# skygazer42/realtime-video-analytics-32streams

Measured on AMD Instinct MI355X. Metric: aggregate detected FPS across streams + p99 per-frame latency, 32x1080p30, higher is better.
Workload: dtype f16

## Files before the change

### include/rva.h

```cpp
#ifndef RVA_H
#define RVA_H

#include <stdint.h>

#ifdef __cplusplus
extern "C" {
#endif

#define RVA_ABI_VERSION 1

enum rva_status {
    RVA_OK = 0,
    RVA_ERR_ARG = 1,
    RVA_ERR_HIP = 2,
    RVA_ERR_CAPACITY = 3,
    RVA_ERR_UNAVAILABLE = 4
};

enum rva_dtype { RVA_F16 = 0, RVA_F32 = 1, RVA_F64 = 2  };

typedef struct rva_ctx rva_ctx;
typedef struct rva_tracker rva_tracker;
typedef void *rva_stream_t;

// ... 147 lines not shown

int rva_sppf_pool3_nhwc_f16(rva_ctx *ctx, const void *in, int ldi, void *out1, void *out2, void *out3, int ldo,
                            int batch, int H, int W, int C, rva_stream_t stream);
int rva_maxpool5_nhwc_f16(rva_ctx *ctx, const void *in, int ldi, void *out, int ldo, int batch, int H,
                          int W, int C, rva_stream_t stream);
int rva_upsample2x_nhwc_f16(rva_ctx *ctx, const void *in, int ldi, void *out, int ldo, int batch, int H,
                            int W, int C, rva_stream_t stream);
int rva_yolo_head_f16(rva_ctx *ctx, const void *box_logits, int ldb, const void *cls_logits, int ldc,
                      void *out, int batch, int h, int w, int nc, int anchors_total, int anchor_offset,
                      float stride, rva_stream_t stream);
int rva_yolo_head3_f16(rva_ctx *ctx, const void *const *box_logits, const int32_t *ldb, const void *const *cls_logits,
                       const int32_t *ldc, void *out, int batch, const int32_t *h, const int32_t *w, int nc,
                       int anchors_total, const float *strides, rva_stream_t stream);
int rva_yolo_head_box32_f16(rva_ctx *ctx, const void *box_logits, int ldb, const void *cls_logits, int ldc, void *out,
                            float *boxes32, int batch, int h, int w, int nc, int anchors_total, int anchor_offset, float stride,
                            rva_stream_t stream);
int rva_yolo_head3_box32_f16(rva_ctx *ctx, const void *const *box_logits, const int32_t *ldb, const void *const *cls_logits,
                             const int32_t *ldc, void *out, float *boxes32, int batch, const int32_t *h, const int32_t *w, int nc,
                             int anchors_total, const float *strides, rva_stream_t stream);
int rva_yolo_head_nc_f16(rva_ctx *ctx, const void *box_logits, int ldb, const void *cls_logits, int ldc, void *out,
                         float *boxes32, int batch, int h, int w, int nc, int anchors_total, int anchor_offset, float stride,
                         rva_stream_t stream);
int rva_yolo_head3_nc_f16(rva_ctx *ctx, const void *const *box_logits, const int32_t *ldb, const void *const *cls_logits,
                          const int32_t *ldc, void *out, float *boxes32, int batch, const int32_t *h, const int32_t *w, int nc,
                          int anchors_total, const float *strides, rva_stream_t stream);
int rva_conv1x1_head_nc_f16(rva_ctx *ctx, const void *in, int ldi, const void *weights, const float *bias, int batch,
                            int H, int W, int Cin, int Cout, int mode, void *out, float *boxes32, int nc, int anchors_total,
                            int anchor_offset, float stride_px, int variant, rva_stream_t stream);

int rva_conv_f32_num_variants(void);
int rva_conv2d_nhwc_f32_v(rva_ctx *ctx, const void *in, int ldi, const void *weights, const float *bias,
                          void *out, int ldo, const void *residual, int ldr, int batch, int H, int W, int Cin,
                          int Cout, int ksize, int stride, int act, int variant, rva_stream_t stream);
int rva_stem_conv_f32(rva_ctx *ctx, const void *in_planar, const void *weights, const float *bias,
                      void *out, int ldo, int batch, int H, int W, int Cout, rva_stream_t stream);
int rva_maxpool5_nhwc_f32(rva_ctx *ctx, const void *in, int ldi, void *out, int ldo, int batch, int H,
                          int W, int C, rva_stream_t stream);
int rva_upsample2x_nhwc_f32(rva_ctx *ctx, const void *in, int ldi, void *out, int ldo, int batch, int H,
                            int W, int C, rva_stream_t stream);
int rva_yolo_head_f32(rva_ctx *ctx, const void *box_logits, int ldb, const void *cls_logits, int ldc,
                      void *out, int batch, int h, int w, int nc, int anchors_total, int anchor_offset,
                      float stride, rva_stream_t stream);

#define RVA_PLAN_NO_STEM2 1
#define RVA_PLAN_NO_CIN_PAD 2
#define RVA_PLAN_NO_PAIR32 4
#define RVA_PLAN_F32 8
#define RVA_PLAN_BOX_F32 16
typedef struct rva_yolov8_plan rva_yolov8_plan;
typedef struct rva_yolov8_desc {
    int32_t batch, height, width;
    int32_t widths[5];
    int32_t depth_backbone[4];
    int32_t depth_head;
    int32_t nc, reg_max;
    int32_t n_convs;
    int32_t flags;
} rva_yolov8_desc;
typedef struct rva_conv_weights {
    const float *weight;
    const float *bias;
    int32_t cout, cin, k, stride;
} rva_conv_weights;
int rva_yolov8_plan_create(rva_ctx *ctx, const rva_yolov8_desc *desc, const rva_conv_weights *convs, rva_yolov8_plan **out);
void rva_yolov8_plan_destroy(rva_yolov8_plan *plan);
int rva_yolov8_plan_info(const rva_yolov8_plan *plan, int32_t *anchors, int32_t *out_rows, int32_t *n_steps, int32_t *n_tunable,
                         int32_t *quiet_step);
int rva_yolov8_plan_output_layout(const rva_yolov8_plan *plan, int64_t *total_bytes, int64_t *boxes_offset);
int rva_yolov8_plan_run(rva_yolov8_plan *plan, const void *input, void *output, rva_stream_t stream);
int rva_yolov8_plan_run_lanes(rva_yolov8_plan *plan, const void *input, void *output, rva_stream_t stream, rva_stream_t side1,
                              rva_stream_t side2);
int rva_yolov8_plan_run_range(rva_yolov8_plan *plan, const void *input, void *output, int first, int last, rva_stream_t stream);
int rva_yolov8_plan_tunable_desc(const rva_yolov8_plan *plan, int index, char *buf, int len);
int rva_yolov8_plan_launch_tunable(rva_yolov8_plan *plan, int index, int variant, void *output, rva_stream_t stream);
int rva_yolov8_plan_set_variant(rva_yolov8_plan *plan, int index, int variant);
int rva_yolov8_plan_get_variant(const rva_yolov8_plan *plan, int index);
int rva_yolov8_plan_set_static_rows(rva_yolov8_plan *plan, int top, int bottom);
int rva_yolov8_plan_run_n(rva_yolov8_plan *plan, const void *input, void *output, int n, rva_stream_t stream);
int rva_yolov8_plan_run_lanes_n(rva_yolov8_plan *plan, const void *input, void *output, int n, rva_stream_t stream, rva_stream_t side1,
                                rva_stream_t side2);
int rva_yolov8_plan_run_range_n(rva_yolov8_plan *plan, const void *input, void *output, int n, int first, int last, rva_stream_t stream);
int rva_yolov8_plan_primed_images(const rva_yolov8_plan *plan);
int rva_yolov8_plan_step_rows(const rva_yolov8_plan *plan, int step, int32_t *y0, int32_t *y1);
int rva_yolov8_plan_step_desc(const rva_yolov8_plan *plan, int step, char *buf, int len);

typedef struct rva_yolov5_desc {
    int32_t batch, height, width;
    int32_t widths[5];
    int32_t depth_backbone[4];
    int32_t depth_head;
    int32_t nc;
    float anchors[18];
    int32_t n_convs;
    int32_t flags;
} rva_yolov5_desc;
int rva_yolov5_plan_create(rva_ctx *ctx, const rva_yolov5_desc *desc, const rva_conv_weights *convs, rva_yolov8_plan **out);
int rva_stem6_conv_f16(rva_ctx *ctx, const void *in_planar, const void *weights, const float *bias, void *out, int ldo,
                       int batch, int H, int W, int Cout, rva_stream_t stream);
int rva_stem6_conv_f16_rows(rva_ctx *ctx, const void *in_planar, const void *weights, const float *bias, void *out, int ldo,
                            int batch, int H, int W, int Cout, int y0, int y1, rva_stream_t stream);
int rva_conv_rows_through_pad(int k, int stride, int pad, int H_in, int lo, int hi, int32_t *out_lo, int32_t *out_hi);
int rva_conv1x1_head5_f16(rva_ctx *ctx, const void *in, int ldi, const void *weights, const float *bias, int batch, int H, int W,
                          int Cin, int nc, const float *anchors_px, void *out, float *boxes32, int anchors_total, int anchor_offset,
                          float stride_px, int variant, rva_stream_t stream);

typedef struct rva_yolo11_desc {
    int32_t batch, height, width;
    int32_t widths[5];
    int32_t repeats[8];
    int32_t c3k[8];
    int32_t psa_blocks, psa_heads;
    int32_t nc;
    int32_t n_convs;
    int32_t flags;
} rva_yolo11_desc;
int rva_yolo11_plan_create(rva_ctx *ctx, const rva_yolo11_desc *desc, const rva_conv_weights *convs, rva_yolov8_plan **out);
int rva_dwconv3x3_nhwc_f16(rva_ctx *ctx, const void *in, int ldi, const void *weights, const float *bias, void *out, int ldo,
                           const void *residual, int ldr, int batch, int H, int W, int C, int act, rva_stream_t stream);
int rva_psa_attention_f16(rva_ctx *ctx, const void *qkv, int ld, void *out, int ldo, int batch, int tokens, int heads,
                          rva_stream_t stream);

typedef struct rva_cnnlstm_plan rva_cnnlstm_plan;
typedef struct rva_cnnlstm_desc {
    int32_t height, width;
    int32_t frames;
    int32_t hidden, classes;
    int32_t max_clips;
} rva_cnnlstm_desc;
typedef struct rva_cnnlstm_weights {
    const float *conv1_w, *conv1_b, *conv2_w, *conv2_b;
    const float *w_ih1, *b1, *w_hh1;
    const float *w_ih2, *w_hh2, *b2;
    const float *head_w, *head_b;
} rva_cnnlstm_weights;
int rva_cnnlstm_plan_create(rva_ctx *ctx, const rva_cnnlstm_desc *desc, const rva_cnnlstm_weights *weights, rva_cnnlstm_plan **out);
void rva_cnnlstm_plan_destroy(rva_cnnlstm_plan *plan);
int rva_cnnlstm_plan_info(const rva_cnnlstm_plan *plan, int32_t *pooled_h, int32_t *pooled_w, int32_t *conv2_tiles,
                          int32_t *n_launches);
int rva_cnnlstm_plan_run(rva_cnnlstm_plan *plan, const void *frames, const int32_t *frame_index, int n_clips, void *logits,
                         rva_stream_t stream);
int rva_cnnlstm_plan_run_post(rva_cnnlstm_plan *plan, const void *logits, const int32_t *rows, int n_rows, int max_det,
                              void *scores, void *cls, void *boxes, void *counts, rva_stream_t stream);
enum rva_cnnlstm_stage {
    RVA_CNNLSTM_STAGE_POOLED = 0, RVA_CNNLSTM_STAGE_PARTIAL = 1, RVA_CNNLSTM_STAGE_FEAT = 2, RVA_CNNLSTM_STAGE_GX = 3,
    RVA_CNNLSTM_STAGE_H1 = 4, RVA_CNNLSTM_STAGE_H2 = 5
};
int rva_cnnlstm_plan_stage(rva_cnnlstm_plan *plan, int stage, int n_clips, void *dst, int64_t dst_floats, int64_t *n_floats,
                           rva_stream_t stream);

typedef struct rva_cnnlstm_f16_plan rva_cnnlstm_f16_plan;
int rva_cnnlstm_f16_plan_create(rva_ctx *ctx, const rva_cnnlstm_desc *desc, const rva_cnnlstm_weights *weights,
                                rva_cnnlstm_f16_plan **out);
void rva_cnnlstm_f16_plan_destroy(rva_cnnlstm_f16_plan *plan);
int rva_cnnlstm_f16_plan_info(const rva_cnnlstm_f16_plan *plan, int32_t *pooled_h, int32_t *pooled_w, int32_t *conv2_tiles,
                              int32_t *n_launches);
int rva_cnnlstm_f16_plan_run(rva_cnnlstm_f16_plan *plan, const void *frames, const int32_t *frame_index, int n_clips, void *logits,
                             rva_stream_t stream);
int rva_cnnlstm_f16_plan_run_post(rva_cnnlstm_f16_plan *plan, const void *logits, const int32_t *rows, int n_rows, int max_det,
                                  void *scores, void *cls, void *boxes, void *counts, rva_stream_t stream);
int rva_cnnlstm_f16_plan_stage(rva_cnnlstm_f16_plan *plan, int stage, int n_clips, void *dst, int64_t dst_elems, int64_t *n_elems,
                               rva_stream_t stream);

typedef struct rva_cnn3d_plan rva_cnn3d_plan;
typedef struct rva_cnn3d_desc {
    int32_t height, width;
    int32_t frames;
// ... 180 lines not shown
```

### realtime_video_analytics_32streams_amd/_native.py

```python
from __future__ import annotations

import ctypes as C
import os
import shutil
import subprocess
from pathlib import Path
from typing import Optional

PKG = Path(__file__).resolve().parent
ROOT = PKG.parent
CSRC = PKG / "csrc"
LIB_PATH = Path(os.environ["RVA_LIB_PATH"]) if os.environ.get("RVA_LIB_PATH") else PKG / "librva.so"
SOURCES = ["rva_ctx.hip", "rva_preprocess.hip", "rva_postprocess.hip", "rva_tracker.hip", "rva_conv.hip", "rva_stem.hip", "rva_yolo_ops.hip", "rva_conv_f32.hip", "rva_attn.hip", "rva_plan.hip", "rva_clip.hip",
           "rva_clip3d.hip", "rva_clip_f16.hip", "rva_resnet.hip", "rva_resnet_f16.hip", "rva_gates.hip", "rva_decode.hip", "rva_preview.hip", "rva_jpeg.hip", "rva_jpeg_dec.hip"]
HIPCC_FLAGS = ["--offload-arch=gfx950", "-O3", "-fPIC", "-shared", "-std=c++17", "-ffp-contract=off",
               "-Wall", "-Wno-unused-function"]

RVA_OK, RVA_ERR_ARG, RVA_ERR_HIP, RVA_ERR_CAPACITY, RVA_ERR_UNAVAILABLE = range(5)
RVA_F16, RVA_F32, RVA_F64 = 0, 1, 2
NORM_IMAGENET_F32, NORM_VIDEO_F32, NORM_IMAGENET_F64 = 0, 1, 2
LAYOUT_NCHW, LAYOUT_CNHW = 0, 1
RVA_MAX_BATCH = 64
RVA_CODEC_H264, RVA_CODEC_HEVC = 0, 1
RVA_JPEG_DEC_BGR, RVA_JPEG_DEC_NV12 = 0, 1
RVA_JPEG_DEC_OK, RVA_JPEG_DEC_REFUSED, RVA_JPEG_DEC_FAILED = 0, -1, -2


class Letterbox(C.Structure):
    _fields_ = [("src_w", C.c_int32), ("src_h", C.c_int32), ("dst_w", C.c_int32), ("dst_h", C.c_int32),
                ("new_w", C.c_int32), ("new_h", C.c_int32), ("pad_left", C.c_int32), ("pad_top", C.c_int32),
                ("scale", C.c_double)]

    def as_meta(self) -> dict:
        return {"orig_shape": (self.src_h, self.src_w), "scale": self.scale, "pad": (self.pad_left, self.pad_top)}


class YoloV8Desc(C.Structure):
    _fields_ = [("batch", C.c_int32), ("height", C.c_int32), ("width", C.c_int32), ("widths", C.c_int32 * 5),
                ("depth_backbone", C.c_int32 * 4), ("depth_head", C.c_int32), ("nc", C.c_int32), ("reg_max", C.c_int32),
                ("n_convs", C.c_int32), ("flags", C.c_int32)]


class YoloV5Desc(C.Structure):
    _fields_ = [("batch", C.c_int32), ("height", C.c_int32), ("width", C.c_int32), ("widths", C.c_int32 * 5),
                ("depth_backbone", C.c_int32 * 4), ("depth_head", C.c_int32), ("nc", C.c_int32), ("anchors", C.c_float * 18),
                ("n_convs", C.c_int32), ("flags", C.c_int32)]


class Yolo11Desc(C.Structure):
    _fields_ = [("batch", C.c_int32), ("height", C.c_int32), ("width", C.c_int32), ("widths", C.c_int32 * 5),
                ("repeats", C.c_int32 * 8), ("c3k", C.c_int32 * 8), ("psa_blocks", C.c_int32), ("psa_heads", C.c_int32),
                ("nc", C.c_int32), ("n_convs", C.c_int32), ("flags", C.c_int32)]


class ConvWeights(C.Structure):
    _fields_ = [("weight", C.POINTER(C.c_float)), ("bias", C.POINTER(C.c_float)), ("cout", C.c_int32), ("cin", C.c_int32),
                ("k", C.c_int32), ("stride", C.c_int32)]


class CnnLstmDesc(C.Structure):
    _fields_ = [("height", C.c_int32), ("width", C.c_int32), ("frames", C.c_int32), ("hidden", C.c_int32), ("classes", C.c_int32),
                ("max_clips", C.c_int32)]


class CnnLstmWeights(C.Structure):
    NAMES = ("conv1_w", "conv1_b", "conv2_w", "conv2_b", "w_ih1", "b1", "w_hh1", "w_ih2", "w_hh2", "b2", "head_w", "head_b")
    _fields_ = [(n, C.POINTER(C.c_float)) for n in NAMES]


class Cnn3dDesc(C.Structure):
    _fields_ = [("height", C.c_int32), ("width", C.c_int32), ("frames", C.c_int32), ("classes", C.c_int32), ("max_clips", C.c_int32)]


class Cnn3dWeights(C.Structure):
    NAMES = ("conv1_w", "conv1_b", "conv2_w", "conv2_b", "conv3_w", "conv3_b", "head_w", "head_b")
    _fields_ = [(n, C.POINTER(C.c_float)) for n in NAMES]


class ResNetDesc(C.Structure):
    _fields_ = [("height", C.c_int32), ("width", C.c_int32), ("classes", C.c_int32), ("top_k", C.c_int32), ("max_frames", C.c_int32)]


class ResNetWeights(C.Structure):
    NAMES = ("stem_w", "stem_b") + tuple(f"c{i}_{x}" for i in range(19) for x in "wb") + ("head_w", "head_b")
    _fields_ = [(n, C.POINTER(C.c_float)) for n in NAMES]


class ResNetConv(C.Structure):
    _fields_ = [("w", C.POINTER(C.c_float)), ("b", C.POINTER(C.c_float))]


class ResNetXDesc(C.Structure):
    _fields_ = [("height", C.c_int32), ("width", C.c_int32), ("classes", C.c_int32), ("top_k", C.c_int32), ("max_frames", C.c_int32),
                ("bottleneck", C.c_int32), ("blocks", C.c_int32 * 4), ("n_convs", C.c_int32), ("flags", C.c_int32)]


# ... 103 lines not shown
        "rva_tracker_update_gated_f32": (C.c_int, [_P, i32p, _P, _P, _P, _P, C.c_int, C.c_double, _P, i32p, _P]),
        "rva_tracker_set_gates": (C.c_int, [_P, i32p, i32p, i32p, i32p, C.c_int]),
        "rva_tracker_snapshot_status": (C.c_int, [_P, C.c_int, _P, _P, C.POINTER(C.c_int32)]),
        "rva_tracker_new_counts": (_P, [_P]),
        "rva_tracker_assign_ids": (C.c_int, [_P, _P, C.c_int, i32p, _P]),
        "rva_tracker_read": (C.c_int, [_P, C.c_int, C.c_int, _P, _P, _P, _P, _P, _P, _P, i32p, _P]),
        "rva_tracker_read_all": (C.c_int, [_P, _P, _P, _P, _P, _P, _P, _P, _P, _P]),
        "rva_tracker_snapshot_async": (C.c_int, [_P, C.c_int, _P]),
        "rva_tracker_snapshot_fetch": (C.c_int, [_P, C.c_int, C.c_int, _P, _P, _P, _P, _P, _P, _P, _P]),
        "rva_tracker_state": (C.c_int, [_P, i64p, C.POINTER(C.c_int), _P]),
        "rva_tracker_set_next_id": (C.c_int, [_P, C.c_int64, _P]),
        "rva_preview_nv12": (C.c_int, [_P, _P, _P, C.c_int, C.c_int, C.c_int, C.c_int, _P, C.c_int, C.c_int, _P, _P, C.c_int, _P, C.c_int,
                                       C.c_int, _P]),
        "rva_decode_available": (C.c_int, [C.c_char_p, C.c_int]),
        "rva_decoder_create": (C.c_int, [_P, C.c_int, C.c_int, C.POINTER(_P)]),
        "rva_decoder_destroy": (None, [_P]),
        "rva_decoder_feed": (C.c_int, [_P, C.c_char_p, C.c_int, C.c_int64, C.c_int]),
        "rva_decoder_next_frame": (C.c_int, [_P, C.POINTER(_P), C.POINTER(_P), i32p, i32p, i32p, i64p, i32p]),
        "rva_decoder_release": (C.c_int, [_P, C.c_int]),
        "rva_motion_nv12_batch": (C.c_int, [_P, pp, pp, i32p, pp, pp, C.c_int, C.c_int, C.c_int, _P, _P]),
        "rva_motion_nv12_masked_batch": (C.c_int, [_P, pp, pp, i32p, pp, pp, pp, C.c_int, C.c_int, C.c_int, _P, _P]),
        "rva_motion_bgr_batch": (C.c_int, [_P, pp, i32p, pp, pp, C.c_int, C.c_int, C.c_int, _P, _P]),
        "rva_preprocess_nv12_masked_batch": (C.c_int, [_P, pp, pp, i32p, pp, C.c_int, C.c_int, C.c_int, _P, C.c_int, C.c_int,
                                                       C.c_int, C.POINTER(Letterbox), _P]),
        "rva_resize_nv12_to_bgr_batch": (C.c_int, [_P, pp, pp, i32p, pp, C.c_int, C.c_int, C.c_int, _P, C.c_int, C.c_int, _P]),
        "rva_tracker_set_box_scale": (C.c_int, [_P, f64p]),
        "rva_conv_cout_pad": (C.c_int, [C.c_int]),
        "rva_conv_num_variants": (C.c_int, []),
        "rva_conv_variant_name": (C.c_char_p, [C.c_int]),
        "rva_conv2d_nhwc_f16": (C.c_int, [_P, _P, C.c_int, _P, _P, _P, C.c_int, _P, C.c_int] + [C.c_int] * 8 + [_P]),
        "rva_conv2d_nhwc_f16_v": (C.c_int, [_P, _P, C.c_int, _P, _P, _P, C.c_int, _P, C.c_int] + [C.c_int] * 9 + [_P]),
        "rva_conv2d_nhwc_f16_rows": (C.c_int, [_P, _P, C.c_int, _P, _P, _P, C.c_int, _P, C.c_int] + [C.c_int] * 11 + [_P]),
        "rva_conv_rows_through": (C.c_int, [C.c_int] * 5 + [i32p, i32p]),
        "rva_stem2_f16_rows": (C.c_int, [_P, _P, _P, _P, _P, _P, _P, C.c_int, C.c_int, C.c_int, C.c_int, C.c_int, C.c_int, _P]),
        "rva_stem_conv_f16": (C.c_int, [_P, _P, _P, _P, _P, C.c_int, C.c_int, C.c_int, C.c_int, C.c_int, _P]),
        "rva_stem2_f16": (C.c_int, [_P, _P, _P, _P, _P, _P, _P, C.c_int, C.c_int, C.c_int, C.c_int, _P]),
        "rva_c2f_pair32_f16": (C.c_int, [_P, _P, C.c_int, _P, _P, _P, _P, _P, C.c_int, C.c_int, C.c_int, C.c_int, _P]),
        "rva_conv1x1_head_f16": (C.c_int, [_P, _P, C.c_int, _P, _P, C.c_int, C.c_int, C.c_int, C.c_int, C.c_int, C.c_int, _P, C.c_int,
                                           C.c_int, C.c_int, C.c_float, C.c_int, _P]),
        "rva_conv1x1_head_box32_f16": (C.c_int, [_P, _P, C.c_int, _P, _P, C.c_int, C.c_int, C.c_int, C.c_int, _P, _P, C.c_int,
                                                 C.c_int, C.c_int, C.c_float, C.c_int, _P]),
        "rva_yolo_head_box32_f16": (C.c_int, [_P, _P, C.c_int, _P, C.c_int, _P, _P, C.c_int, C.c_int, C.c_int, C.c_int, C.c_int,
                                              C.c_int, C.c_float, _P]),
        "rva_yolo_head3_box32_f16": (C.c_int, [_P, pp, i32p, pp, i32p, _P, _P, C.c_int, i32p, i32p, C.c_int, C.c_int,
                                               C.POINTER(C.c_float), _P]),
        "rva_yolo_head_nc_f16": (C.c_int, [_P, _P, C.c_int, _P, C.c_int, _P, _P, C.c_int, C.c_int, C.c_int, C.c_int, C.c_int,
                                           C.c_int, C.c_float, _P]),
        "rva_yolo_head3_nc_f16": (C.c_int, [_P, pp, i32p, pp, i32p, _P, _P, C.c_int, i32p, i32p, C.c_int, C.c_int,
                                            C.POINTER(C.c_float), _P]),
        "rva_conv1x1_head_nc_f16": (C.c_int, [_P, _P, C.c_int, _P, _P, C.c_int, C.c_int, C.c_int, C.c_int, C.c_int, C.c_int, _P, _P,
                                              C.c_int, C.c_int, C.c_int, C.c_float, C.c_int, _P]),
        "rva_conv1x1_upcat_f16": (C.c_int, [_P, _P, C.c_int, C.c_int, _P, C.c_int, C.c_int, _P, _P, _P, C.c_int, C.c_int, C.c_int,
                                            C.c_int, C.c_int, C.c_int, C.c_int, _P]),
        "rva_yolo_head3_f16": (C.c_int, [_P, pp, i32p, pp, i32p, _P, C.c_int, i32p, i32p, C.c_int, C.c_int, C.POINTER(C.c_float), _P]),
        "rva_sppf_pool3_nhwc_f16": (C.c_int, [_P, _P, C.c_int, _P, _P, _P, C.c_int, C.c_int, C.c_int, C.c_int, C.c_int, _P]),
        "rva_maxpool5_nhwc_f16": (C.c_int, [_P, _P, C.c_int, _P, C.c_int, C.c_int, C.c_int, C.c_int, C.c_int, _P]),
        "rva_upsample2x_nhwc_f16": (C.c_int, [_P, _P, C.c_int, _P, C.c_int, C.c_int, C.c_int, C.c_int, C.c_int, _P]),
        "rva_yolo_head_f16": (C.c_int, [_P, _P, C.c_int, _P, C.c_int, _P, C.c_int, C.c_int, C.c_int, C.c_int, C.c_int,
                                        C.c_int, C.c_float, _P]),
        "rva_conv_f32_num_variants": (C.c_int, []),
        "rva_conv2d_nhwc_f32_v": (C.c_int, [_P, _P, C.c_int, _P, _P, _P, C.c_int, _P, C.c_int] + [C.c_int] * 9 + [_P]),
        "rva_stem_conv_f32": (C.c_int, [_P, _P, _P, _P, _P, C.c_int, C.c_int, C.c_int, C.c_int, C.c_int, _P]),
        "rva_maxpool5_nhwc_f32": (C.c_int, [_P, _P, C.c_int, _P, C.c_int, C.c_int, C.c_int, C.c_int, C.c_int, _P]),
        "rva_upsample2x_nhwc_f32": (C.c_int, [_P, _P, C.c_int, _P, C.c_int, C.c_int, C.c_int, C.c_int, C.c_int, _P]),
        "rva_yolo_head_f32": (C.c_int, [_P, _P, C.c_int, _P, C.c_int, _P, C.c_int, C.c_int, C.c_int, C.c_int, C.c_int,
                                        C.c_int, C.c_float, _P]),
        "rva_yolov8_plan_create": (C.c_int, [_P, C.POINTER(YoloV8Desc), C.POINTER(ConvWeights), C.POINTER(_P)]),
        "rva_yolov8_plan_destroy": (None, [_P]),
        "rva_yolov8_plan_info": (C.c_int, [_P, i32p, i32p, i32p, i32p, i32p]),
        "rva_yolov8_plan_output_layout": (C.c_int, [_P, i64p, i64p]),
        "rva_yolov8_plan_run": (C.c_int, [_P, _P, _P, _P]),
        "rva_yolov8_plan_run_lanes": (C.c_int, [_P, _P, _P, _P, _P, _P]),
        "rva_yolov8_plan_run_range": (C.c_int, [_P, _P, _P, C.c_int, C.c_int, _P]),
        "rva_yolov8_plan_tunable_desc": (C.c_int, [_P, C.c_int, C.c_char_p, C.c_int]),
        "rva_yolov8_plan_launch_tunable": (C.c_int, [_P, C.c_int, C.c_int, _P, _P]),
        "rva_yolov8_plan_set_variant": (C.c_int, [_P, C.c_int, C.c_int]),
        "rva_yolov8_plan_get_variant": (C.c_int, [_P, C.c_int]),
        "rva_yolov8_plan_set_static_rows": (C.c_int, [_P, C.c_int, C.c_int]),
        "rva_yolov8_plan_step_rows": (C.c_int, [_P, C.c_int, i32p, i32p]),
        "rva_yolov8_plan_run_n": (C.c_int, [_P, _P, _P, C.c_int, _P]),
        "rva_yolov8_plan_run_lanes_n": (C.c_int, [_P, _P, _P, C.c_int, _P, _P, _P]),
        "rva_yolov8_plan_run_range_n": (C.c_int, [_P, _P, _P, C.c_int, C.c_int, C.c_int, _P]),
        "rva_yolov8_plan_primed_images": (C.c_int, [_P]),
        "rva_yolov5_plan_create": (C.c_int, [_P, C.POINTER(YoloV5Desc), C.POINTER(ConvWeights), C.POINTER(_P)]),
        "rva_stem6_conv_f16": (C.c_int, [_P, _P, _P, _P, _P, C.c_int, C.c_int, C.c_int, C.c_int, C.c_int, _P]),
        "rva_stem6_conv_f16_rows": (C.c_int, [_P, _P, _P, _P, _P, C.c_int, C.c_int, C.c_int, C.c_int, C.c_int, C.c_int, C.c_int, _P]),
        "rva_conv_rows_through_pad": (C.c_int, [C.c_int] * 6 + [i32p, i32p]),
        "rva_conv1x1_head5_f16": (C.c_int, [_P, _P, C.c_int, _P, _P, C.c_int, C.c_int, C.c_int, C.c_int, C.c_int, _P, _P, _P,
                                            C.c_int, C.c_int, C.c_float, C.c_int, _P]),
        "rva_yolov8_plan_step_desc": (C.c_int, [_P, C.c_int, C.c_char_p, C.c_int]),
        "rva_yolo11_plan_create": (C.c_int, [_P, C.POINTER(Yolo11Desc), C.POINTER(ConvWeights), C.POINTER(_P)]),
        "rva_dwconv3x3_nhwc_f16": (C.c_int, [_P, _P, C.c_int, _P, _P, _P, C.c_int, _P, C.c_int] + [C.c_int] * 5 + [_P]),
        "rva_psa_attention_f16": (C.c_int, [_P, _P, C.c_int, _P, C.c_int, C.c_int, C.c_int, C.c_int, _P]),
        "rva_cnnlstm_plan_create": (C.c_int, [_P, C.POINTER(CnnLstmDesc), C.POINTER(CnnLstmWeights), C.POINTER(_P)]),
        "rva_cnnlstm_plan_destroy": (None, [_P]),
        "rva_cnnlstm_plan_info": (C.c_int, [_P, i32p, i32p, i32p, i32p]),
        "rva_cnnlstm_plan_run": (C.c_int, [_P, _P, _P, C.c_int, _P, _P]),
        "rva_cnnlstm_plan_run_post": (C.c_int, [_P, _P, _P, C.c_int, C.c_int, _P, _P, _P, _P, _P]),
        "rva_cnnlstm_plan_stage": (C.c_int, [_P, C.c_int, C.c_int, _P, C.c_int64, i64p, _P]),
        "rva_cnnlstm_f16_plan_create": (C.c_int, [_P, C.POINTER(CnnLstmDesc), C.POINTER(CnnLstmWeights), C.POINTER(_P)]),
        "rva_cnnlstm_f16_plan_destroy": (None, [_P]),
        "rva_cnnlstm_f16_plan_info": (C.c_int, [_P, i32p, i32p, i32p, i32p]),
        "rva_cnnlstm_f16_plan_run": (C.c_int, [_P, _P, _P, C.c_int, _P, _P]),
        "rva_cnnlstm_f16_plan_run_post": (C.c_int, [_P, _P, _P, C.c_int, C.c_int, _P, _P, _P, _P, _P]),
        "rva_cnnlstm_f16_plan_stage": (C.c_int, [_P, C.c_int, C.c_int, _P, C.c_int64, i64p, _P]),
        "rva_cnn3d_plan_create": (C.c_int, [_P, C.POINTER(Cnn3dDesc), C.POINTER(Cnn3dWeights), C.POINTER(_P)]),
        "rva_cnn3d_plan_destroy": (None, [_P]),
        "rva_cnn3d_plan_info": (C.c_int, [_P, i32p, i32p, i32p, i32p]),
        "rva_cnn3d_plan_run": (C.c_int, [_P, _P, _P, C.c_int, _P, _P]),
        "rva_cnn3d_plan_run_post": (C.c_int, [_P, _P, _P, C.c_int, C.c_int, _P, _P, _P, _P, _P]),
        "rva_cnn3d_plan_stage": (C.c_int, [_P, C.c_int, C.c_int, _P, C.c_int64, i64p, _P]),
        "rva_cnn3d_f16_plan_create": (C.c_int, [_P, C.POINTER(Cnn3dDesc), C.POINTER(Cnn3dWeights), C.POINTER(_P)]),
        "rva_cnn3d_f16_plan_destroy": (None, [_P]),
        "rva_cnn3d_f16_plan_info": (C.c_int, [_P, i32p, i32p, i32p, i32p]),
        "rva_cnn3d_f16_plan_run": (C.c_int, [_P, _P, _P, C.c_int, _P, _P]),
        "rva_cnn3d_f16_plan_run_post": (C.c_int, [_P, _P, _P, C.c_int, C.c_int, _P, _P, _P, _P, _P]),
        "rva_cnn3d_f16_plan_stage": (C.c_int, [_P, C.c_int, C.c_int, _P, C.c_int64, i64p, _P]),
        "rva_resnet_plan_create": (C.c_int, [_P, C.POINTER(ResNetDesc), C.POINTER(ResNetWeights), C.POINTER(_P)]),
        "rva_resnet_plan_destroy": (None, [_P]),
        "rva_resnet_plan_info": (C.c_int, [_P, i32p, i64p, i32p]),
        "rva_resnet_plan_run": (C.c_int, [_P, _P, _P, C.c_int, _P, _P]),
        "rva_resnet_plan_run_post": (C.c_int, [_P, _P, _P, C.c_int, C.c_int, _P, _P, _P, _P, _P]),
        "rva_resnet_plan_stage": (C.c_int, [_P, C.c_int, C.c_int, _P, C.c_int64, i64p, _P]),
        "rva_resnet_f16_plan_create": (C.c_int, [_P, C.POINTER(ResNetDesc), C.POINTER(ResNetWeights), C.POINTER(_P)]),
        "rva_resnet_f16_plan_destroy": (None, [_P]),
        "rva_resnet_f16_plan_info": (C.c_int, [_P, i32p, i64p, i32p]),
        "rva_resnet_f16_plan_run": (C.c_int, [_P, _P, _P, C.c_int, _P, _P]),
        "rva_resnet_f16_plan_run_post": (C.c_int, [_P, _P, _P, C.c_int, C.c_int, _P, _P, _P, _P, _P]),
        "rva_resnet_f16_plan_stage": (C.c_int, [_P, C.c_int, C.c_int, _P, C.c_int64, i64p, _P]),
        "rva_resnetx_f16_plan_create": (C.c_int, [_P, C.POINTER(ResNetXDesc), C.POINTER(ResNetXWeights), C.POINTER(_P)]),
        "rva_resnetx_f16_plan_destroy": (None, [_P]),
        "rva_resnetx_f16_plan_info": (C.c_int, [_P, i32p, i64p, i32p]),
        "rva_resnetx_f16_plan_run": (C.c_int, [_P, _P, _P, C.c_int, _P, _P]),
        "rva_resnetx_f16_plan_run_post": (C.c_int, [_P, _P, _P, C.c_int, C.c_int, _P, _P, _P, _P, _P]),
        "rva_resnetx_f16_plan_stage": (C.c_int, [_P, C.c_int, C.c_int, _P, C.c_int64, i64p, _P]),
        "rva_jpeg_max_bytes": (C.c_int, [C.c_int, C.c_int]),
        "rva_jpeg_encode_bgr": (C.c_int, [_P, _P, C.c_int, C.c_int, C.c_int, C.c_int, _P, C.c_int, _P, _P]),
        "rva_jpeg_status": (C.c_int, [_P, _P, C.POINTER(C.c_int)]),
        "rva_jpeg_batch_create": (C.c_int, [_P, C.c_int, C.c_int, C.c_int, C.POINTER(_P)]),
        "rva_jpeg_batch_destroy": (None, [_P]),
        "rva_jpeg_batch_encode": (C.c_int, [_P, C.c_int, pp, i32p, i32p, i32p, i32p, _P, C.c_int64, _P, _P]),
        "rva_preview_nv12_batch": (C.c_int, [_P, _P, _P, C.c_int64, C.c_int, C.c_int, C.c_int, C.c_int, _P]),
        "rva_jpeg_dec_probe": (C.c_int, [C.c_char_p, C.c_int64, C.POINTER(JpegDecInfo), C.c_char_p, C.c_int]),
        "rva_jpeg_dec_create": (C.c_int, [_P, C.c_int, C.c_int, C.c_int, C.c_int, C.POINTER(_P)]),
        "rva_jpeg_dec_destroy": (None, [_P]),
        "rva_jpeg_dec_decode": (C.c_int, [_P, C.c_int, C.POINTER(C.c_char_p), i64p, C.c_int, pp, pp, i32p, _P]),
        "rva_jpeg_dec_status": (C.c_int, [_P, i32p]),
        "rva_jpeg_dec_times": (C.c_int, [_P, f32p]),
    }
    for name, (res, args) in sig.items():
        fn = getattr(L, name)
        fn.restype = res
        fn.argtypes = args
    if L.rva_abi_version() != 1:
        raise RuntimeError("librva.so ABI version mismatch; rebuild it")
    _LIB = L
    return L


EXPORTS = [
    "rva_abi_version", "rva_create", "rva_destroy", "rva_last_error", "rva_reserve", "rva_letterbox_meta",
    "rva_preprocess_nv12_batch", "rva_preprocess_nv12_content_batch", "rva_preprocess_bgr_batch", "rva_preprocess_clip_nv12_batch",
    "rva_preprocess_clip_bgr_batch", "rva_profile_next_preprocess", "rva_preprocess_frames_nv12_batch", "rva_preprocess_frames_bgr_batch", "rva_postprocess_batch", "rva_post_status", "rva_post_filter_stats", "rva_tracker_create",
    "rva_tracker_destroy", "rva_tracker_update_f32", "rva_tracker_update_f64", "rva_tracker_update_gated_f32",
    "rva_tracker_set_gates", "rva_tracker_snapshot_status", "rva_tracker_new_counts",
    "rva_tracker_assign_ids", "rva_tracker_read", "rva_tracker_read_all", "rva_tracker_snapshot_async",
    "rva_tracker_snapshot_fetch", "rva_tracker_state",
    "rva_tracker_set_next_id", "rva_preview_nv12", "rva_decode_available", "rva_decoder_create", "rva_decoder_destroy", "rva_decoder_feed",
    "rva_decoder_next_frame", "rva_decoder_release", "rva_motion_nv12_batch", "rva_motion_nv12_masked_batch", "rva_motion_bgr_batch",
    "rva_preprocess_nv12_masked_batch", "rva_resize_nv12_to_bgr_batch", "rva_tracker_set_box_scale", "rva_conv_cout_pad", "rva_conv_num_variants", "rva_conv_variant_name", "rva_conv2d_nhwc_f16", "rva_conv2d_nhwc_f16_v", "rva_stem_conv_f16", "rva_stem2_f16", "rva_c2f_pair32_f16",
    "rva_conv1x1_head_f16", "rva_conv1x1_upcat_f16", "rva_sppf_pool3_nhwc_f16", "rva_maxpool5_nhwc_f16", "rva_upsample2x_nhwc_f16", "rva_yolo_head_f16", "rva_yolo_head3_f16",
    "rva_conv_f32_num_variants", "rva_conv2d_nhwc_f32_v", "rva_stem_conv_f32", "rva_maxpool5_nhwc_f32", "rva_upsample2x_nhwc_f32",
    "rva_yolo_head_f32",
    "rva_postprocess_boxes_batch", "rva_conv1x1_head_box32_f16", "rva_yolo_head_box32_f16", "rva_yolo_head3_box32_f16",
    "rva_yolo_head_nc_f16", "rva_yolo_head3_nc_f16", "rva_conv1x1_head_nc_f16",
    "rva_yolov8_plan_output_layout",
    "rva_yolov8_plan_create", "rva_yolov8_plan_destroy", "rva_yolov8_plan_info", "rva_yolov8_plan_run", "rva_yolov8_plan_run_lanes",
    "rva_yolov8_plan_run_range", "rva_yolov8_plan_tunable_desc", "rva_yolov8_plan_launch_tunable", "rva_yolov8_plan_set_variant",
    "rva_yolov8_plan_get_variant", "rva_yolov8_plan_set_static_rows", "rva_yolov8_plan_step_rows", "rva_yolov8_plan_run_n",
    "rva_yolov8_plan_run_lanes_n", "rva_yolov8_plan_run_range_n", "rva_yolov8_plan_primed_images", "rva_conv2d_nhwc_f16_rows",
    "rva_stem2_f16_rows", "rva_conv_rows_through", "rva_cnnlstm_plan_create", "rva_cnnlstm_plan_destroy", "rva_cnnlstm_plan_info", "rva_cnnlstm_plan_run",
    "rva_cnnlstm_plan_run_post", "rva_cnnlstm_plan_stage", "rva_cnnlstm_f16_plan_create", "rva_cnnlstm_f16_plan_destroy", "rva_cnnlstm_f16_plan_info",
    "rva_cnnlstm_f16_plan_run", "rva_cnnlstm_f16_plan_run_post", "rva_cnnlstm_f16_plan_stage", "rva_cnn3d_plan_create", "rva_cnn3d_plan_destroy", "rva_cnn3d_plan_info", "rva_cnn3d_plan_run",
    "rva_cnn3d_plan_run_post", "rva_cnn3d_plan_stage", "rva_cnn3d_f16_plan_create", "rva_cnn3d_f16_plan_destroy", "rva_cnn3d_f16_plan_info",
    "rva_cnn3d_f16_plan_run", "rva_cnn3d_f16_plan_run_post", "rva_cnn3d_f16_plan_stage", "rva_resnet_plan_create", "rva_resnet_plan_destroy", "rva_resnet_plan_info",
    "rva_resnet_plan_run", "rva_resnet_plan_run_post", "rva_resnet_plan_stage", "rva_resnet_f16_plan_create", "rva_resnet_f16_plan_destroy",
    "rva_resnet_f16_plan_info", "rva_resnet_f16_plan_run", "rva_resnet_f16_plan_run_post", "rva_resnet_f16_plan_stage", "rva_jpeg_max_bytes", "rva_jpeg_encode_bgr", "rva_jpeg_status",
    "rva_jpeg_batch_create", "rva_jpeg_batch_destroy", "rva_jpeg_batch_encode", "rva_preview_nv12_batch",
    "rva_yolov5_plan_create", "rva_stem6_conv_f16", "rva_stem6_conv_f16_rows", "rva_conv_rows_through_pad", "rva_conv1x1_head5_f16",
    "rva_yolo11_plan_create", "rva_dwconv3x3_nhwc_f16", "rva_psa_attention_f16", "rva_yolov8_plan_step_desc",
    "rva_resnetx_f16_plan_create", "rva_resnetx_f16_plan_destroy", "rva_resnetx_f16_plan_info", "rva_resnetx_f16_plan_run",
    "rva_resnetx_f16_plan_run_post", "rva_resnetx_f16_plan_stage",
    "rva_jpeg_dec_probe", "rva_jpeg_dec_create", "rva_jpeg_dec_destroy", "rva_jpeg_dec_decode", "rva_jpeg_dec_status", "rva_jpeg_dec_times",
]


class Context:

    def __init__(self, device: int = 0):
        L = lib()
        h = _P()
        rc = L.rva_create(device, C.byref(h))
        if rc != RVA_OK or not h:
            raise RuntimeError(
                f"rva_create(device={device}) failed with status {rc}: no usable HIP device. "
                "The MI355X hot path has no CPU fallback.")
        self.handle = h
        self.device = device

    def check(self, rc: int, what: str = "") -> None:
        if rc != RVA_OK:
            msg = lib().rva_last_error(self.handle)
            raise RuntimeError(f"{what or 'librva'} failed (status {rc}): {msg.decode() if msg else ''}")

    def close(self) -> None:
        if getattr(self, "handle", None):
            lib().rva_destroy(self.handle)
            self.handle = None

    def __del__(self):
        try:
            self.close()
        except Exception:
            pass


def letterbox(src_w: int, src_h: int, dst_w: int, dst_h: int) -> Letterbox:
    m = Letterbox()
    rc = lib().rva_letterbox_meta(src_w, src_h, dst_w, dst_h, C.byref(m))
    if rc != RVA_OK:
        raise ValueError(f"bad letterbox geometry {(src_w, src_h)} -> {(dst_w, dst_h)}")
    return m


def ptr_array(ptrs):
    arr = (_P * len(ptrs))(*[_P(int(p)) for p in ptrs])
    return C.cast(arr, C.POINTER(_P)), arr


def i32_array(vals):
    arr = (C.c_int32 * len(vals))(*[int(v) for v in vals])
    return C.cast(arr, C.POINTER(C.c_int32)), arr
```

### realtime_video_analytics_32streams_amd/csrc/rva_conv.hip

```cpp
#include "rva_conv_dev.h"

namespace {

struct ConvArgs {
    const __half *in; int ldi;
    const __half *w;
    const float *bias;
    __half *out; int ldo;
    union {
        const __half *res;
        float *hbox;
    };
    int ldr;
    int CoutPad;
    __half *hout; int hmode, hnc, hA, ha0, hW, hHW; float hstride;
    union {
        const __half *in2;
        const float *hanc;
    };
    int ldi2, c_split;
    int H, W, Cin, CinPad, Ho, Wo, Cout, stride, M, act, n_tiles, m_tiles;
    int wy0, wrows;
};

__device__ __forceinline__ int div_s(int q, int d, float inv)
{
    int t = (int)((float)q * inv);
    const int r = q - t * d;
    if (r < 0) --t;
    if (r >= d) ++t;
    return t;
}

__device__ __forceinline__ int tap_mask9(int ox, int oy, int W, int H)
{
    const int hv = (ox >= 1 ? 1 : 0) | 2 | (ox <= W - 2 ? 4 : 0);
    return (oy >= 1 ? hv : 0) | (hv << 3) | (oy <= H - 2 ? hv << 6 : 0);
}
__device__ __forceinline__ int raster_tap_mask9(int p, int M, int HW, int W, int H, float inv_hw, float inv_w)
{
    if (p >= M) return 0;
    const int rem = p - div_s(p, HW, inv_hw) * HW, oy = div_s(rem, W, inv_w), ox = rem - oy * W;
    return tap_mask9(ox, oy, W, H);
}


template <int FN> __device__ __forceinline__ float4 bias_frag(const float4 (&bvs)[FN], int i, int) { return bvs[i]; }
__device__ __forceinline__ float4 bias_frag(const float *bias, int i, int lane) { return *reinterpret_cast<const float4 *>(bias + (16 * i + (lane >> 4) * 4)); }

template <int BN, int TM, int TN, int FM, int FN, class A, class Bias>
__device__ __forceinline__ void stage_tile(const f4 (&acc)[FN][FM], const A &a, const Bias &bias, int wm, int wn, int lane)
{
    constexpr int SROW = BN + 8;
    extern __shared__ __attribute__((aligned(16))) unsigned char smem[];
    __half *stage = (__half *)smem;
#pragma unroll
    for (int i = 0; i < FN; ++i) {
        const int co = wn * TN + 16 * i + (lane >> 4) * 4;
        const float4 bv = bias_frag(bias, i, lane);
#pragma unroll
        for (int j = 0; j < FM; ++j) {
            float v0 = acc[i][j][0] + bv.x, v1 = acc[i][j][1] + bv.y, v2 = acc[i][j][2] + bv.z, v3 = acc[i][j][3] + bv.w;
            if (a.act) { v0 = silu_f(v0); v1 = silu_f(v1); v2 = silu_f(v2); v3 = silu_f(v3); }
            const int px = wm * TM + 16 * j + (lane & 15);
            __half2 lo = __floats2half2_rn(v0, v1), hi = __floats2half2_rn(v2, v3);
            uint2 pk;
            pk.x = *reinterpret_cast<uint32_t *>(&lo);
            pk.y = *reinterpret_cast<uint32_t *>(&hi);
            *reinterpret_cast<uint2 *>(stage + (size_t)px * SROW + co) = pk;
        }
    }
}

template <int BM, int BN, int NT, class A, class Map>
__device__ __forceinline__ void store_tile(const A &a, int n0, int tid, Map map)
{
    constexpr int SROW = BN + 8, CPR = BN / 8;
    extern __shared__ __attribute__((aligned(16))) unsigned char smem[];
    const __half *stage = (const __half *)smem;
#pragma unroll 4
    for (int q = tid; q < BM * CPR; q += NT) {
        const int row = q / CPR, pc = q - row * CPR;
        const int co = n0 + pc * 8;
        size_t m;
        if (map(row, m) && co < a.Cout) {
            uint4 v = *reinterpret_cast<const uint4 *>(stage + (size_t)row * SROW + pc * 8);
            if (a.res) {
                const uint4 r = *reinterpret_cast<const uint4 *>(a.res + m * a.ldr + co);
                __half2 *vh = reinterpret_cast<__half2 *>(&v);
                const __half2 *rh = reinterpret_cast<const __half2 *>(&r);
#pragma unroll
                for (int u = 0; u < 4; ++u) {
                    const float2 x = __half22float2(vh[u]), y = __half22float2(rh[u]);
                    vh[u] = __floats2half2_rn(x.x + y.x, x.y + y.y);
                }
            }
            *reinterpret_cast<uint4 *>(a.out + m * a.ldo + co) = v;
        }
    }
}

template <int BN, int WPX, int KS, int BK>
__global__ void __launch_bounds__(256) k_conv_mfma(ConvArgs a)
// ... 1308 lines not shown
        wait_vm_n(NSLOT >= 3 ? min(max(nsteps - 1 - sf, 0), NSLOT - 2) * my_pieces : 0);
        __builtin_amdgcn_s_barrier();
        const int sn = (sf + NSLOT - 1) * SUB;
        const bool more = sn < nsteps;
        const bool early = NSLOT == 2 || wv < 4;
        if (early) {
#pragma unroll
            for (int u = 0; u < SUB; ++u)
                if (sn + u < nsteps) GB_ISSUE();
        }
#pragma unroll
      for (int u = 0; u < SUB; ++u) {
        const int s = sf * SUB + u;
        if (SUB > 1 && s >= nsteps) break;
        const int tap = s / cpt;
        const __half *ab = ring + (size_t)(s % (NSLOT * SUB)) * SLOTH;
        const __half *wb = ab + BM * BK;
        const int arow = wm * TM + (lane & 15), wr = wn * TN + (lane & 15);
#pragma unroll
        for (int ks = 0; ks < BK / 32; ++ks) {
            h8 bf[FM];
#pragma unroll
            for (int j = 0; j < FM; ++j) {
                const int r = arow + 16 * j;
                bf[j] = *reinterpret_cast<const h8 *>(ab + (BK == 64 ? r * 64 + ((ks * 4 + (lane >> 4)) ^ xr) * 8 : swz32(r, lane >> 4)));
                if (KS == 3 && !((vm[j] >> tap) & 1)) bf[j] = hz;
            }
#pragma unroll
            for (int i = 0; i < FN; ++i) {
                const int r = wr + 16 * i;
                const h8 af = *reinterpret_cast<const h8 *>(wb + (BK == 64 ? r * 64 + ((ks * 4 + (lane >> 4)) ^ xr) * 8 : swz32(r, lane >> 4)));
#pragma unroll
                for (int j = 0; j < FM; ++j) acc[i][j] = __builtin_amdgcn_mfma_f32_16x16x32_f16(af, bf[j], acc[i][j], 0, 0, 0);
            }
        }
      }
        if (more && !early) GB_ISSUE();
    }
#undef GB_ISSUE
    __syncthreads();

    stage_tile<BN, TM, TN>(acc, a, bvs, wm, wn, lane);
    __syncthreads();
    if constexpr (HEAD) {
        constexpr int SROW = BN + 8;
        const __half *stage = (const __half *)smem;
        if (a.hmode == 3) {
            const int no = 5 + a.hnc, creal = 3 * no;
            const float aw[3] = {a.hanc[0], a.hanc[2], a.hanc[4]}, ah[3] = {a.hanc[1], a.hanc[3], a.hanc[5]};
            const int groups = (min(BN, a.Cout - n0) + 7) >> 3;
            for (int q = tid; q < BM * groups; q += 512) {
                const int cg = q / BM, r = q - cg * BM;
                const int m = P0 + r;
                if (m >= a.M) continue;
                const int b = m / a.hHW, i = m - b * a.hHW;
                const float gx = (float)(i % a.hW), gy = (float)(i / a.hW);
                const uint4 qv = *reinterpret_cast<const uint4 *>(stage + (size_t)r * SROW + cg * 8);
                const __half *zh = reinterpret_cast<const __half *>(&qv);
                const int c0 = n0 + cg * 8;
                int an = c0 / no, j = c0 - an * no;
#pragma unroll
                for (int e = 0; e < 8; ++e) {
                    if (c0 + e < creal) {
                        const float y = __builtin_amdgcn_rcpf(1.0f + __expf(-__half2float(zh[e])));
                        float v = y;
                        if (j < 2) v = (y * 2.0f - 0.5f + (j == 0 ? gx : gy)) * a.hstride;
                        else if (j < 4) { const float t2 = y * 2.0f; v = t2 * t2 * (j == 2 ? (an == 0 ? aw[0] : an == 1 ? aw[1] : aw[2]) : (an == 0 ? ah[0] : an == 1 ? ah[1] : ah[2])); }
                        const size_t at = (size_t)a.ha0 + (size_t)an * a.hHW + i;
                        a.hout[((size_t)b * no + j) * a.hA + at] = __float2half_rn(v);
                        if (j < 4 && a.hbox) a.hbox[((size_t)b * 4 + j) * a.hA + at] = v;
                    }
                    if (++j == no) { j = 0; ++an; }
                }
            }
            return;
        }
        for (int r = tid; r < BM; r += 512) {
            const int m = P0 + r;
            if (m >= a.M) continue;
            const int b = m / a.hHW, i = m - b * a.hHW;
            __half *o = a.hout + (size_t)b * (4 + a.hnc) * a.hA + a.ha0 + i;
            const __half *row = stage + (size_t)r * SROW;
            if (a.hmode == 1) {
                float d[4];
#pragma unroll
                for (int sd = 0; sd < 4; ++sd) {
                    float v[16], mx = -1e30f;
                    const uint4 q0 = *reinterpret_cast<const uint4 *>(row + sd * 16), q1 = *reinterpret_cast<const uint4 *>(row + sd * 16 + 8);
                    const __half2 *h0 = reinterpret_cast<const __half2 *>(&q0), *h1 = reinterpret_cast<const __half2 *>(&q1);
#pragma unroll
                    for (int t = 0; t < 4; ++t) {
                        float2 f = __half22float2(h0[t]); v[2 * t] = f.x; v[2 * t + 1] = f.y;
                        f = __half22float2(h1[t]); v[8 + 2 * t] = f.x; v[9 + 2 * t] = f.y;
                    }
#pragma unroll
                    for (int t = 0; t < 16; ++t) mx = fmaxf(mx, v[t]);
                    float se = 0.f, sw = 0.f;
#pragma unroll
                    for (int t = 0; t < 16; ++t) { const float e = __expf(v[t] - mx); se += e; sw += e * (float)t; }
                    d[sd] = sw / se;
                }
                const float ax = (float)(i % a.hW) + 0.5f, ay = (float)(i / a.hW) + 0.5f;
                const float x1 = ax - d[0], y1 = ay - d[1], x2 = ax + d[2], y2 = ay + d[3];
                o[0] = __float2half_rn((x1 + x2) * 0.5f * a.hstride);
                o[(size_t)a.hA] = __float2half_rn((y1 + y2) * 0.5f * a.hstride);
                o[(size_t)2 * a.hA] = __float2half_rn((x2 - x1) * a.hstride);
                o[(size_t)3 * a.hA] = __float2half_rn((y2 - y1) * a.hstride);
                if (a.hbox) {
                    float *o32 = a.hbox + (size_t)b * 4 * a.hA + a.ha0 + i;
                    o32[0] = (x1 + x2) * 0.5f * a.hstride;
                    o32[(size_t)a.hA] = (y1 + y2) * 0.5f * a.hstride;
                    o32[(size_t)2 * a.hA] = (x2 - x1) * a.hstride;
                    o32[(size_t)3 * a.hA] = (y2 - y1) * a.hstride;
                }
            } else {
                const int cend = min(BN, a.Cout - n0);
                for (int c = 0; c < cend; c += 8) {
                    const uint4 q = *reinterpret_cast<const uint4 *>(row + c);
                    const int k = n0 + c;
                    if (k + 8 <= a.hnc) store_scores8<false>(o + (size_t)(4 + k) * a.hA, (size_t)a.hA, q, 8);
                    else store_scores8<true>(o + (size_t)(4 + k) * a.hA, (size_t)a.hA, q, a.hnc - k);
                }
            }
        }
        return;
    }
    const int wskip = (a.Ho - a.wrows) * a.Wo;
    const int M = a.M, wfirst = a.wy0 * a.Wo;
    store_tile<BM, BN, 512>(a, n0, tid, [=](int row, size_t &m) {
        const int mw = P0 + row;
        m = (size_t)(wskip ? mw + div_s(mw, HoWo, inv_howo) * wskip + wfirst : mw);
        return mw < M;
    });
}

template <int BM, int BN, int WGM, int WGN, int NSLOT, int KS, int BK, bool UP = false, bool HEAD = false, int SUB = 1>
hipError_t launch_gbig1(ConvArgs &a, hipStream_t s)
{
    constexpr size_t smem = ldsdma_smem((size_t)NSLOT * SUB * (BM + BN) * BK * 2, BM, BN);
    static_assert(smem <= 160 * 1024, "LDS budget");
    return launch_ldsdma(k_conv_gbig<BM, BN, WGM, WGN, NSLOT, KS, BK, UP, HEAD, SUB>, a, BM, BN, a.M, (size_t)a.H * a.W * (size_t)(a.M / (a.wrows * a.Wo) + 1),
                         UP ? a.ldi2 : a.ldi, (size_t)a.CoutPad * KS * KS * a.Cin, smem, smem, s);
}

template <int BM, int BN, int WGM, int WGN, int NSLOT, int BK = 64, int SUB = 1>
hipError_t launch_gbig(ConvArgs &a, int ksize, hipStream_t s)
{
    if (a.Cin % BK || a.H > 2000 || a.W > 2000) return hipErrorInvalidValue;
    return ksize == 1 ? launch_gbig1<BM, BN, WGM, WGN, NSLOT, 1, BK, false, false, SUB>(a, s)
                      : launch_gbig1<BM, BN, WGM, WGN, NSLOT, 3, BK, false, false, SUB>(a, s);
}

struct S2Args {
    const __half *in; int ldi;
    const __half *w; const float *bias;
    __half *out; int ldo;
    const __half *res; int ldr;
    int B, H, W, Ho, Wo, Cout, CoutPad, act, tiles_x, tiles_y, total, n_tiles;
    int y0, y1;
};

template <int STRIDE, int CIN, int CO, int NWV, int NBUF, int RPW = 1>
__global__ void __launch_bounds__(NWV * 64) k_conv3_patch(S2Args a)
{
    static_assert(CIN == 32 || CIN == 64, "input channels");
    constexpr int TH = NWV * RPW, TW = 32, NT = NWV * 64, FMW = 2 * RPW;
    constexpr int PH = STRIDE == 2 ? 2 * TH + 1 : TH + 2;
    constexpr int CW = STRIDE == 2 ? TW + 1 : TW + 2;
    constexpr int PROWS = STRIDE == 2 ? PH * 2 * CW : PH * CW;
    constexpr int RPP = 512 / CIN, LPR = CIN / 8;
    constexpr int PPIECES = (PROWS + RPP - 1) / RPP;
    constexpr int WPIECES = 9 * CO / RPP;
    constexpr int FN = CO / 16, KCH = CIN / 32;
    constexpr int SROW = CO + 8;
    static_assert(TH * TW * SROW * 2 <= PPIECES * 1024, "the output stage reuses a patch buffer");
    extern __shared__ __attribute__((aligned(16))) unsigned char smem[];
    __half *wl = (__half *)smem;
    __half *patch0 = wl + WPIECES * 512;
    const int tid = threadIdx.x, lane = tid & 63;
    const int wv = __builtin_amdgcn_readfirstlane(tid >> 6);
    const int lrow = lane / LPR, lp = lane % LPR;
    const int tiles_img = a.tiles_x * a.tiles_y;
    const int n0 = (int)(blockIdx.x % a.n_tiles) * CO;
    const int bid = blockIdx.x / a.n_tiles, nblk = gridDim.x / a.n_tiles;
    auto src_c8 = [&](int row) { return (CIN == 64 ? (lp ^ (row & 7)) : ((lp - 2 * (row >> 2)) & 3)) * 8; };
    auto lds_off = [&](int row, int c) { return CIN == 64 ? row * 64 + ((c ^ (row & 7)) << 3) : swz32(row, c); };

    float4 bvs[FN];
#pragma unroll
    for (int i = 0; i < FN; ++i) bvs[i] = *reinterpret_cast<const float4 *>(a.bias + min(n0 + 16 * i + (lane >> 4) * 4, a.CoutPad - 4));

#pragma unroll
    for (int k = 0; k < (WPIECES + NWV - 1) / NWV; ++k) {
        const int idx = wv + NWV * k;
        if (idx < WPIECES) {
            const int row = idx * RPP + lrow;
            const int tap = row / CO, co = min(n0 + row - tap * CO, a.CoutPad - 1);
            const __half *src = a.w + (size_t)(co * 9 + tap) * CIN + src_c8(row);
            __builtin_amdgcn_global_load_lds((glb_vptr)src, (lds_vptr)(wl + idx * 512), 16, 0, 0);
        }
    }
    constexpr int NPP = (PPIECES + NWV - 1) / NWV;
    int pdy[NPP], pdx[NPP], pc8[NPP];
#pragma unroll
// ... 876 lines not shown

extern "C" {

int rva_conv2d_nhwc_f16(rva_ctx *ctx, const void *in, int ldi, const void *weights, const float *bias, void *out,
                        int ldo, const void *residual, int ldr, int batch, int H, int W, int Cin, int Cout, int ksize,
                        int stride, int act, rva_stream_t stream_)
{
    return rva_conv2d_nhwc_f16_v(ctx, in, ldi, weights, bias, out, ldo, residual, ldr, batch, H, W, Cin, Cout, ksize, stride,
                                 act, 0, stream_);
}

int rva_conv2d_nhwc_f16_v(rva_ctx *ctx, const void *in, int ldi, const void *weights, const float *bias, void *out,
                          int ldo, const void *residual, int ldr, int batch, int H, int W, int Cin, int Cout, int ksize,
                          int stride, int act, int variant, rva_stream_t stream_)
{
    return rva_conv2d_nhwc_f16_sel(ctx, in, ldi, weights, bias, out, ldo, residual, ldr, batch, batch, H, W, Cin, Cout, ksize, stride, act,
                                   variant, 0, -1, stream_);
}

int rva_conv2d_nhwc_f16_rows(rva_ctx *ctx, const void *in, int ldi, const void *weights, const float *bias, void *out,
                             int ldo, const void *residual, int ldr, int batch, int H, int W, int Cin, int Cout, int ksize,
                             int stride, int act, int variant, int y0, int y1, rva_stream_t stream_)
{
    return rva_conv2d_nhwc_f16_sel(ctx, in, ldi, weights, bias, out, ldo, residual, ldr, batch, batch, H, W, Cin, Cout, ksize, stride, act,
                                   variant, y0, y1, stream_);
}

}

int rva_conv2d_nhwc_f16_sel(rva_ctx *ctx, const void *in, int ldi, const void *weights, const float *bias, void *out,
                            int ldo, const void *residual, int ldr, int batch, int sel_batch, int H, int W, int Cin, int Cout, int ksize,
                            int stride, int act, int variant, int y0, int y1, rva_stream_t stream_)
{
    if (!ctx) return RVA_ERR_ARG;
    const ConvVariant *row = find_variant(variant);
    if (!in || !weights || !bias || !out || batch <= 0 || sel_batch < batch || H <= 0 || W <= 0 || (ksize != 1 && ksize != 3) ||
        (stride != 1 && stride != 2) || Cin % 8 || Cout % 8 || ldi % 8 || ldo % 8 || (residual && ldr % 8) || !row ||
        ((uintptr_t)in | (uintptr_t)out | (uintptr_t)weights | (uintptr_t)residual) % 16)
        return rva_fail(ctx, RVA_ERR_ARG, "rva_conv2d_nhwc_f16: unsupported shape/alignment (Cin%%8, Cout%%8, ld%%8, 16-byte pointers)");
    ConvCall c{};
    ConvArgs &a = c.a;
    a.in = (const __half *)in; a.ldi = ldi; a.w = (const __half *)weights; a.bias = bias;
    a.out = (__half *)out; a.ldo = ldo; a.res = (const __half *)residual; a.ldr = ldr;
    a.H = H; a.W = W; a.Cin = Cin; a.CinPad = rva_ceil_div(Cin, 32) * 32; a.Cout = Cout; a.stride = stride; a.act = act;
    const int pad = ksize / 2;
    a.Ho = (H + 2 * pad - ksize) / stride + 1;
    a.Wo = (W + 2 * pad - ksize) / stride + 1;
    a.M = batch * a.Ho * a.Wo;
    a.wy0 = 0; a.wrows = a.Ho;
    if (rva_row_window(ctx, "rva_conv2d_nhwc_f16_rows", y0, y1, a.Ho)) return RVA_ERR_ARG;
    c.y0 = y0; c.y1 = y1;
    c.batch = batch; c.sel_batch = sel_batch; c.ksize = ksize;
    c.cpad = rva_ceil_div(Cout, 64) * 64;
    c.num_cus = rva_num_cus(ctx);
    c.s = (hipStream_t)stream_;
    const hipError_t ev = row->launch(c);
    if (ev == hipSuccess) return RVA_OK;
    (void)hipGetLastError();
    if (ev == hipErrorInvalidValue) return rva_fail(ctx, RVA_ERR_ARG, "conv variant %d not applicable here", variant);
    return rva_fail(ctx, RVA_ERR_HIP, "conv variant %d: launch failed: %s", variant, hipGetErrorString(ev));
}

extern "C" {

int rva_conv1x1_upcat_f16(rva_ctx *ctx, const void *low, int ld_low, int c_low, const void *skip, int ld_skip, int c_skip,
                          const void *weights, const float *bias, void *out, int ldo, int batch, int H, int W, int Cout,
                          int act, int variant, rva_stream_t stream_)
{
    if (!ctx) return RVA_ERR_ARG;
    if (!low || !skip || !weights || !bias || !out || batch <= 0 || H <= 0 || W <= 0 || (H | W) & 1 || c_low <= 0 || c_skip <= 0 ||
        c_low % 64 || c_skip % 64 || Cout % 8 || ld_low % 8 || ld_skip % 8 || ldo % 8 ||
        ((uintptr_t)low | (uintptr_t)skip | (uintptr_t)out | (uintptr_t)weights) % 16 || H > 2000 || W > 2000)
        return rva_fail(ctx, RVA_ERR_ARG, "rva_conv1x1_upcat_f16: unsupported shape/alignment (even H, W; channel counts %% 64; ld %% 8)");
    ConvArgs a{};
    a.in = (const __half *)low; a.ldi = ld_low; a.in2 = (const __half *)skip; a.ldi2 = ld_skip; a.c_split = c_low;
    a.w = (const __half *)weights; a.bias = bias; a.out = (__half *)out; a.ldo = ldo; a.res = nullptr; a.ldr = 0;
    a.H = H; a.W = W; a.Cin = c_low + c_skip; a.CinPad = a.Cin; a.Cout = Cout; a.stride = 1; a.act = act;
    a.Ho = H; a.Wo = W; a.M = batch * H * W; a.CoutPad = rva_ceil_div(Cout, 64) * 64; a.wy0 = 0; a.wrows = H;
    return launch_gather64_1x1<true, false>(ctx, "rva_conv1x1_upcat_f16", a, variant, (hipStream_t)stream_);
}

static int conv1x1_head(rva_ctx *ctx, const void *in, int ldi, const void *weights, const float *bias, int batch, int H, int W,
                        int Cin, int Cout, int mode, void *out, float *boxes32, int nc, int anchors_total, int anchor_offset, float stride_px,
                        int variant, rva_stream_t stream_, bool any_nc = false)
{
    if (!ctx) return RVA_ERR_ARG;
    if (any_nc && (nc < 1 || nc > 1024 || anchor_offset < 0 || H <= 0 || W <= 0 || anchor_offset + H * W > anchors_total ||
                   (boxes32 && ((uintptr_t)boxes32 % 4 || mode != 1))))
        return rva_fail(ctx, RVA_ERR_ARG, "rva_conv1x1_head_nc_f16: 1 <= nc <= 1024, the level inside the anchor range, boxes32 (mode 1) a float tensor");
    if (!in || !weights || !bias || !out || batch <= 0 || H <= 0 || W <= 0 || Cin % 64 || Cout % 8 || ldi % 8 || (!any_nc && nc % 8) ||
        (mode != 1 && mode != 2) || (mode == 1 && Cout != 64) || (mode == 2 && Cout != (nc + 7) / 8 * 8) ||
        ((uintptr_t)in | (uintptr_t)weights) % 16 || H > 2000 || W > 2000)
        return rva_fail(ctx, RVA_ERR_ARG, "rva_conv1x1_head_f16: unsupported shape (Cin %% 64; box branch Cout = 64; class branch Cout = nc, rounded up to 8 by _nc)");
    ConvArgs a{};
    a.in = (const __half *)in; a.ldi = ldi; a.w = (const __half *)weights; a.bias = bias; a.out = nullptr; a.ldo = 0;
    a.H = H; a.W = W; a.Cin = Cin; a.CinPad = Cin; a.Cout = Cout; a.stride = 1; a.act = 0; a.Ho = H; a.Wo = W; a.M = batch * H * W;
    a.CoutPad = rva_ceil_div(Cout, 64) * 64; a.wy0 = 0; a.wrows = H;
    a.hout = (__half *)out; a.hmode = mode; a.hnc = nc; a.hA = anchors_total; a.ha0 = anchor_offset; a.hW = W; a.hHW = H * W;
    a.hstride = stride_px;
    a.hbox = boxes32;
    return launch_gather64_1x1<false, true>(ctx, "rva_conv1x1_head_f16", a, variant, (hipStream_t)stream_);
}

int rva_conv1x1_head_f16(rva_ctx *ctx, const void *in, int ldi, const void *weights, const float *bias, int batch, int H, int W,
                         int Cin, int Cout, int mode, void *out, int nc, int anchors_total, int anchor_offset, float stride_px,
                         int variant, rva_stream_t stream_)
{
    return conv1x1_head(ctx, in, ldi, weights, bias, batch, H, W, Cin, Cout, mode, out, nullptr, nc, anchors_total, anchor_offset, stride_px, variant, stream_);
}

int rva_conv1x1_head_box32_f16(rva_ctx *ctx, const void *in, int ldi, const void *weights, const float *bias, int batch, int H, int W,
                               int Cin, void *out, float *boxes32, int nc, int anchors_total, int anchor_offset, float stride_px,
                               int variant, rva_stream_t stream_)
{
    if (!ctx) return RVA_ERR_ARG;
    if (!boxes32 || (uintptr_t)boxes32 % 4 || anchor_offset < 0 || anchor_offset + H * W > anchors_total)
        return rva_fail(ctx, RVA_ERR_ARG, "rva_conv1x1_head_box32_f16: boxes32 must be a float tensor [batch, 4, anchors_total] and the level must lie inside it");
    return conv1x1_head(ctx, in, ldi, weights, bias, batch, H, W, Cin, 64, 1, out, boxes32, nc, anchors_total, anchor_offset, stride_px, variant, stream_);
}

int rva_conv1x1_head_nc_f16(rva_ctx *ctx, const void *in, int ldi, const void *weights, const float *bias, int batch, int H, int W,
                            int Cin, int Cout, int mode, void *out, float *boxes32, int nc, int anchors_total, int anchor_offset,
                            float stride_px, int variant, rva_stream_t stream_)
{
    return conv1x1_head(ctx, in, ldi, weights, bias, batch, H, W, Cin, Cout, mode, out, boxes32, nc, anchors_total, anchor_offset, stride_px, variant,
                        stream_, true);
}

int rva_conv1x1_head5_f16(rva_ctx *ctx, const void *in, int ldi, const void *weights, const float *bias, int batch, int H, int W,
                          int Cin, int nc, const float *anchors_px, void *out, float *boxes32, int anchors_total, int anchor_offset,
                          float stride_px, int variant, rva_stream_t stream_)
{
    if (!ctx) return RVA_ERR_ARG;
    if (!in || !weights || !bias || !out || !anchors_px || batch <= 0 || H <= 0 || W <= 0 || H > 2000 || W > 2000 || Cin <= 0 || Cin % 64 ||
        ldi % 8 || ldi < Cin || nc < 1 || nc > 1024 || anchor_offset < 0 || (long)anchor_offset + 3l * H * W > anchors_total ||
        ((uintptr_t)in | (uintptr_t)weights) % 16 || (uintptr_t)out % 2 || ((uintptr_t)boxes32 | (uintptr_t)anchors_px | (uintptr_t)bias) % 4)
        return rva_fail(ctx, RVA_ERR_ARG, "rva_conv1x1_head5_f16: Cin %% 64 == 0, ldi %% 8 == 0, 1 <= nc <= 1024, the level's 3*H*W anchors inside "
                                          "the anchor range, 16-byte aligned input and weights");
    const int Cout = (3 * (5 + nc) + 7) / 8 * 8;
    ConvArgs a{};
    a.in = (const __half *)in; a.ldi = ldi; a.w = (const __half *)weights; a.bias = bias; a.out = nullptr; a.ldo = 0;
    a.H = H; a.W = W; a.Cin = Cin; a.CinPad = Cin; a.Cout = Cout; a.stride = 1; a.act = 0; a.Ho = H; a.Wo = W; a.M = batch * H * W;
    a.CoutPad = rva_ceil_div(Cout, 64) * 64; a.wy0 = 0; a.wrows = H;
    a.hout = (__half *)out; a.hmode = 3; a.hnc = nc; a.hA = anchors_total; a.ha0 = anchor_offset; a.hW = W; a.hHW = H * W;
    a.hstride = stride_px;
    a.hbox = boxes32;
    a.hanc = anchors_px;
    return launch_gather64_1x1<false, true>(ctx, "rva_conv1x1_head5_f16", a, variant, (hipStream_t)stream_);
}

int rva_conv_cout_pad(int Cout) { return rva_ceil_div(Cout, 64) * 64; }

int rva_conv_num_variants(void) { return RVA_CONV_VARIANTS; }

const char *rva_conv_variant_name(int variant)
{
    const ConvVariant *row = find_variant(variant);
    return row ? row->name : nullptr;
}

}
```

### realtime_video_analytics_32streams_amd/csrc/rva_conv_dev.h

```cpp
#pragma once

#include <hip/hip_fp16.h>

#include <cstdlib>

#include "rva_internal.h"

namespace {

typedef _Float16 h8 __attribute__((ext_vector_type(8)));
typedef float f4 __attribute__((ext_vector_type(4)));
typedef unsigned int u4 __attribute__((ext_vector_type(4)));

#ifdef RVA_ROW_STAMPS
#define RVA_DBG_FIELD int dbg;
#define RVA_DBG(a, bit) ((a).dbg & (bit))
#else
#define RVA_DBG_FIELD
#define RVA_DBG(a, bit) 0
#endif
#ifdef RVA_ROW_STAMPS
__device__ unsigned long long g_stamps[8][256];
__device__ __forceinline__ unsigned long long stamp_now()
{
    unsigned long long t;
    asm volatile("s_memtime %0\n\ts_waitcnt lgkmcnt(0)" : "=s"(t)::"memory");
    return t;
}
#define STAMP(k) do { if (st_on && st_n < 256) g_stamps[st_slot][st_n++] = stamp_now(); } while (0)
#define STAMP_BEGIN_ON(WHO, DIV, NB, SLOT)                                                                                 \
    const int st_stride = gridDim.x / (DIV);                                                                               \
    const bool st_on = (WHO) && st_stride > 0 && blockIdx.x % st_stride == 0 && blockIdx.x / st_stride < (NB);             \
    const int st_slot = st_on ? (SLOT) : 0;                                                                                \
    int st_n = 0
#define RVA_STAMP_READER(name) \
    extern "C" int name(unsigned long long *host) { return (int)hipMemcpyFromSymbol(host, HIP_SYMBOL(g_stamps), sizeof(unsigned long long) * 8 * 256); }
#else
#define STAMP(k) do { } while (0)
#define STAMP_BEGIN_ON(WHO, DIV, NB, SLOT) do { } while (0)
#endif
#define STAMP_BEGIN() STAMP_BEGIN_ON(tid == 0, 8, 8, blockIdx.x / st_stride)

__device__ __forceinline__ int swz32(int row, int chunk) { return row * 32 + (((chunk + 2 * (row >> 2)) & 3) << 3); }

__device__ __forceinline__ float silu_f(float v) { return v * __builtin_amdgcn_rcpf(1.0f + __expf(-v)); }

typedef __attribute__((address_space(3))) void *lds_vptr;
typedef const __attribute__((address_space(1))) void *glb_vptr;

template <int N> __device__ __forceinline__ void wait_vm() { asm volatile("s_waitcnt vmcnt(%0)" ::"n"(N) : "memory"); }

template <bool GUARD>
__device__ __forceinline__ void store_scores8(__half *o, size_t A, const uint4 q, int left)
{
    const __half2 *hq = reinterpret_cast<const __half2 *>(&q);
#pragma unroll
    for (int t = 0; t < 4; ++t) {
        const float2 f = __half22float2(hq[t]);
        if (!GUARD || 2 * t < left) o[(size_t)(2 * t) * A] = __float2half_rn(__builtin_amdgcn_rcpf(1.0f + __expf(-f.x)));
        if (!GUARD || 2 * t + 1 < left) o[(size_t)(2 * t + 1) * A] = __float2half_rn(__builtin_amdgcn_rcpf(1.0f + __expf(-f.y)));
    }
}

}
```

### realtime_video_analytics_32streams_amd/csrc/rva_internal.h

```cpp
#pragma once

#include <hip/hip_runtime.h>

#include <algorithm>
#include <cstdarg>
#include <cstdint>
#include <cstdio>
#include <map>
#include <string>
#include <vector>

#include "rva.h"

struct rva_resize_table {
    int32_t *ofs = nullptr;
    int16_t *w0 = nullptr;
    int16_t *w1 = nullptr;
    int n = 0;
};

struct rva_geom_cache {
    rva_resize_table x, y;
};

struct rva_jpeg_state;

struct rva_ctx {
    int device = 0;
    rva_jpeg_state *jpeg = nullptr;
    std::string err;
    int cap_batch = 0, cap_anchors = 0;
    float *sp_box = nullptr;
    float *sp_score = nullptr;
    int32_t *sp_cls = nullptr;
    uint32_t *cand_bits = nullptr;
    int32_t *post_flags = nullptr;
    std::map<uint64_t, rva_resize_table> taps_x, taps_y;
    hipEvent_t k1_start = nullptr, k1_stop = nullptr;
    int k1_px = -1;
    int k1_nt = -1;
    int num_cus = 0;
};

inline int rva_fail(rva_ctx *ctx, int code, const char *fmt, ...)
{
    char buf[512];
    va_list ap;
    va_start(ap, fmt);
    vsnprintf(buf, sizeof buf, fmt, ap);
    va_end(ap);
    if (ctx) ctx->err = buf;
    return code;
}

#define RVA_HIP(ctx, call)                                                                          \
    do {                                                                                            \
        hipError_t e_ = (call);                                                                     \
        if (e_ != hipSuccess)                                                                       \
            return rva_fail((ctx), RVA_ERR_HIP, "%s failed: %s (%s:%d)", #call, hipGetErrorString(e_), \
                            __FILE__, __LINE__);                                                    \
    } while (0)

int rva_get_taps(rva_ctx *ctx, int src, int dst, bool is_x, rva_resize_table *out);

static inline int rva_ceil_div(int a, int b) { return (a + b - 1) / b; }

inline int rva_row_window(rva_ctx *ctx, const char *who, int y0, int &y1, int Ho)
{
    if (y1 < 0) y1 = Ho;
    if (y0 < 0 || y0 >= y1 || y1 > Ho) return rva_fail(ctx, RVA_ERR_ARG, "%s: rows [%d, %d) are not a window of %d output rows", who, y0, y1, Ho);
    return RVA_OK;
}

hipError_t rva_func_smem(const void *fn, size_t bytes);

int rva_num_cus(rva_ctx *ctx);

bool rva_conv_variant_is_gather64(int variant);
bool rva_conv_variant_rows(int variant, int Cin, int ksize, int stride);

int rva_conv2d_nhwc_f16_sel(rva_ctx *ctx, const void *in, int ldi, const void *weights, const float *bias, void *out, int ldo,
                            const void *residual, int ldr, int batch, int sel_batch, int H, int W, int Cin, int Cout, int ksize, int stride,
                            int act, int variant, int y0, int y1, rva_stream_t stream);

void rva_jpeg_free(rva_ctx *ctx);


struct rva_dev_arena {
    std::vector<void *> allocs;

    template <typename T>
    int alloc(rva_ctx *ctx, T **dst, size_t n)
    {
        void *m = nullptr;
        RVA_HIP(ctx, hipMalloc(&m, std::max<size_t>(n, 1) * sizeof(T)));
        allocs.push_back(m);
        *dst = (T *)m;
        return RVA_OK;
    }

    template <typename T>
    int upload(rva_ctx *ctx, T **dst, const T *src, size_t n)
    {
        const int rc = alloc(ctx, dst, n);
        if (rc != RVA_OK) return rc;
        RVA_HIP(ctx, hipMemcpy(*dst, src, n * sizeof(T), hipMemcpyHostToDevice));
        return RVA_OK;
    }

    void release()
    {
        for (void *m : allocs) (void)hipFree(m);
        allocs.clear();
    }
};

int rva_plan_fits(rva_ctx *ctx, const char *who, size_t need, const char *shape);

constexpr int RVA_PLAN_MAX_CLASSES = 16384;

inline int rva_half_map(int n, int k, int pad) { return (n + 2 * pad - k) / 2 + 1; }
inline void rva_stem_maps(int H, int W, int *Hc, int *Wc, int *Hp, int *Wp)
{
    *Hc = rva_half_map(H, 7, 3); *Wc = rva_half_map(W, 7, 3);
    *Hp = rva_half_map(*Hc, 3, 1); *Wp = rva_half_map(*Wc, 3, 1);
}

template <typename T>
std::vector<T> rva_pack_taps_major(const T *w, int cout, int cin)
{
    std::vector<T> out((size_t)cout * 9 * cin);
    for (int co = 0; co < cout; ++co)
        for (int ci = 0; ci < cin; ++ci)
            for (int t = 0; t < 9; ++t) out[((size_t)co * 9 + t) * cin + ci] = w[((size_t)co * cin + ci) * 9 + t];
    return out;
}

int rva_clip_stem_prepare(rva_ctx *ctx);
int rva_clip_stem_launch(rva_ctx *ctx, const float *frames, const int32_t *frame_index, const float *w1, const float *b1, float *pooled,
                         int H, int W, int n_frames, hipStream_t st);
int rva_clip_mean_launch(rva_ctx *ctx, const float *partial, int tiles, float n, float *feat, int rows, int channels, hipStream_t st);
int rva_clip_head_prepare(rva_ctx *ctx, int hidden);
int rva_clip_head_launch(rva_ctx *ctx, const float *x, const float *wh, const float *bh, float *logits, int hidden, int classes,
                         int n_clips, hipStream_t st);
int rva_clip_post_prepare(rva_ctx *ctx, int classes);
int rva_clip_post_launch(rva_ctx *ctx, const char *who, const float *logits, int classes, int k, const int32_t *rows, int n_rows,
                         int max_det, float *scores, int32_t *cls, float *boxes, int32_t *counts, hipStream_t st);

bool rva_round_f16(const float *src, size_t n, std::vector<_Float16> &dst);
std::vector<_Float16> rva_clip16_stem_pack(const std::vector<_Float16> &c1);
int rva_clip16_stem_prepare(rva_ctx *ctx);
int rva_clip16_stem_launch(rva_ctx *ctx, const _Float16 *frames, const int32_t *frame_index, const _Float16 *w1, const float *b1,
                           _Float16 *pooled, int H, int W, int n_frames, hipStream_t st);

int rva_res_mean_launch(rva_ctx *ctx, const float *x, int P, int C, float *feat, int n, hipStream_t st);

int rva_clip_stage_copy(rva_ctx *ctx, const char *who, int stage, int n, const char *items, const void *src, size_t esize,
                        const char *unit, int64_t count, int64_t rows, int64_t row_elems, int64_t pitch_elems, void *dst,
                        int64_t dst_elems, int64_t *n_elems, hipStream_t st);
```

### realtime_video_analytics_32streams_amd/csrc/rva_plan.hip

```cpp
#include <algorithm>
#include <cstring>
#include <deque>
#include <memory>

#include "rva_internal.h"

namespace {

enum StepKind { K_CONV, K_UPCAT, K_HEAD, K_STEM2, K_STEM, K_SPPF3, K_POOL5, K_UP2, K_HEAD3, K_PAIR32,
                K_CONV_F32, K_STEM_F32, K_POOL5_F32, K_UP2_F32, K_HEAD_F32, K_STEM6, K_HEAD5, K_DWCONV, K_ATTN };

struct View {
    char *base = nullptr; int ld = 0, off = 0, ch = 0, es = 2;
    void *ptr() const { return base + (size_t)es * off; }
    View sub(int o, int c) const { View v = *this; v.off += o; v.ch = c; return v; }
};

struct Step {
    StepKind kind;
    int lane = 0;
    int tunable = -1;
    const void *in = nullptr, *in2 = nullptr; int ldi = 0, ldi2 = 0, c_in = 0, c_in2 = 0;
    const void *w = nullptr, *w2 = nullptr; const float *b = nullptr, *b2 = nullptr;
    void *out = nullptr, *out2 = nullptr, *out3 = nullptr; int ldo = 0;
    const void *res = nullptr; int ldr = 0;
    int H = 0, W = 0, Cin = 0, Cout = 0, k = 0, stride = 0, act = 0, variant = 0;
    int mode = 0, a0 = 0; float stride_px = 0.f;
    int c_real = 0;
    int Ho = 0, y0 = 0, y1 = 0;
    const void *hb[3] = {nullptr, nullptr, nullptr}, *hk[3] = {nullptr, nullptr, nullptr};
    int32_t hldb[3] = {0, 0, 0}, hldc[3] = {0, 0, 0}, hh[3] = {0, 0, 0}, hw[3] = {0, 0, 0}; float hs[3] = {0, 0, 0};
};

struct Tunable { int step; std::string base, desc; };

}

struct rva_yolov8_plan {
    rva_ctx *ctx = nullptr;
    rva_yolov8_desc d{};
    int B = 0, H = 0, W = 0, nc = 0, A = 0;
    int head_rows = 0;
    std::vector<void *> allocs;
    std::vector<Step> steps;
    std::vector<Tunable> tunables;
    int fork_step[3] = {-1, -1, -1};
    int quiet_step = 0;
    hipEvent_t fork_ev[3] = {nullptr, nullptr, nullptr}, join_ev[3] = {nullptr, nullptr, nullptr};
    bool fused_stem = false, fused_head = false;
    bool f32 = false;
    bool box32 = false;
    size_t box_off = 0;
    int rows_top = 0, rows_bottom = 0;
    bool windowed = false;
    int primed = 0;
};

namespace {

struct Geo {
    int B = 0, H = 0, W = 0, c[6] = {}, h[6] = {}, w[6] = {};
    explicit Geo(const rva_yolov8_desc &d) : B(d.batch), H(d.height), W(d.width)
    {
        for (int l = 1; l <= 5; ++l) { c[l] = d.widths[l - 1]; h[l] = H >> l; w[l] = W >> l; }
    }
    float stride(int l) const { return (float)(1 << l); }
    int a0(int l) const { return l <= 3 ? 0 : a0(l - 1) + h[l - 1] * w[l - 1]; }
};

struct Src {
    View v, low; bool up = false;
    Src(View x) : v(x) {}
    Src(View l, View skip) : v(skip), low(l), up(true) {}
    int ch() const { return up ? low.ch + v.ch : v.ch; }
};

struct Head {
    int rm4, cb, cc_real, cc, ncp;
    const rva_conv_weights *box[3][3];
    Step h3s;
};

struct Builder {
    rva_yolov8_plan *p;
    const rva_conv_weights *convs;
    const Geo g;
    int next = 0;
    int lane = 0;
    int fork_at[2] = {-1, -1};
    std::string err;
    bool hip_failed = false;
    std::deque<std::vector<float>> pad_store;
    std::deque<rva_conv_weights> pad_convs;

    Builder(rva_yolov8_plan *plan, const rva_conv_weights *cv) : p(plan), convs(cv), g(plan->d) {}

    bool fail(const std::string &m, bool hip = false)
    {
        if (err.empty()) { err = m; hip_failed = hip; }
        return false;
    }

    void *dev_alloc(size_t bytes, bool zero)
    {
        void *ptr = nullptr;
        if (hipMalloc(&ptr, bytes ? bytes : 16) != hipSuccess) { fail("hipMalloc failed", true); return nullptr; }
        p->allocs.push_back(ptr);
        if (zero && hipMemset(ptr, 0, bytes) != hipSuccess) { fail("hipMemset failed", true); return nullptr; }
        return ptr;
    }
    View buf(int l, int ch)
    {
        View v;
        v.es = p->f32 ? 4 : 2;
        v.base = (char *)dev_alloc((size_t)g.B * g.h[l] * g.w[l] * ch * v.es + 64, true);
        v.ld = ch; v.off = 0; v.ch = ch;
        return v;
    }
    bool upload(const void *host, size_t bytes, const void **dev, const char *what = "weight")
    {
        void *d = dev_alloc(bytes, false);
        if (!d) return false;
        if (hipMemcpy(d, host, bytes, hipMemcpyHostToDevice) != hipSuccess) return fail(std::string(what) + " upload failed", true);
        *dev = d;
        return true;
    }
    bool upload(const void *w, size_t w_bytes, const std::vector<float> &b, const void **dw, const float **db, const char *what = "weight")
    {
        const void *d = nullptr;
        if (!upload(w, w_bytes, dw, what) || !upload(b.data(), b.size() * sizeof(float), &d, what)) return false;
        *db = (const float *)d;
        return true;
    }
    template <typename T>
    bool pack_as(const rva_conv_weights *const *cv, int n, bool pad, Step &s, bool second)
    {
        if (!err.empty()) return false;
        const rva_conv_weights &c0 = *cv[0];
// ... 307 lines not shown
    bool bottom_up(Block block, View n3, View cat4, View cat5, View feats[3], const char *const what[4])
    {
        const View cat[2] = {cat4, cat5};
        feats[0] = n3; feats[1] = buf(4, g.c[4]); feats[2] = buf(5, g.c[5]);
        for (int i = 0; i < 2; ++i) {
            const View x = feats[i];
            fork_at[i] = (int)p->steps.size();
            if (!conv1(take(x.ch, x.ch, 3, 2, what[2 * i]), x, cat[i].sub(0, x.ch), 3 + i, 1)) return false;
            if (!block(6 + i, cat[i], feats[i + 1], 4 + i, what[2 * i + 1])) return false;
        }
        return true;
    }
    bool head_open(Head &hd)
    {
        const int nc = p->d.nc, ncm = nc < 100 ? nc : 100, cal = p->f32 ? 16 : 8;
        hd.rm4 = 4 * p->d.reg_max;
        hd.cb = std::max(g.c[3] / 4, hd.rm4);
        hd.cc_real = std::max(g.c[3], ncm);
        hd.cc = (hd.cc_real + cal - 1) / cal * cal; hd.ncp = (nc + 7) / 8 * 8;
        hd.h3s = Step{}; hd.h3s.kind = K_HEAD3;
        p->A = g.a0(6);
        p->fused_head = !p->f32 && hd.cb % 64 == 0 && hd.cc % 64 == 0 && hd.rm4 == 64;
        for (int l = 0; l < 3; ++l) {
            hd.box[l][0] = take(g.c[3 + l], hd.cb, 3, 1, "detect.box.0"); hd.box[l][1] = take(hd.cb, hd.cb, 3, 1, "detect.box.1");
            hd.box[l][2] = take(hd.cb, hd.rm4, 1, 1, "detect.box.2");
            if (!hd.box[l][0] || !hd.box[l][1] || !hd.box[l][2]) return false;
        }
        return true;
    }
    bool head_last(Head &hd, int l, int mode, const rva_conv_weights *c, View src)
    {
        if (p->fused_head) return head(c, src, mode, l);
        View o = buf(l, mode == 1 ? hd.rm4 : hd.ncp);
        if (!conv1(c, src, o, l, 0)) return false;
        Step &h = hd.h3s;
        const int i = l - 3;
        (mode == 1 ? h.hb : h.hk)[i] = o.ptr(); (mode == 1 ? h.hldb : h.hldc)[i] = o.ld; h.hh[i] = g.h[l]; h.hw[i] = g.w[l]; h.hs[i] = g.stride(l);
        if (p->f32 && mode == 2) {
            Step s{}; s.kind = K_HEAD_F32; s.in = h.hb[i]; s.ldi = h.hldb[i]; s.in2 = h.hk[i]; s.ldi2 = h.hldc[i];
            s.H = g.h[l]; s.W = g.w[l]; s.a0 = g.a0(l); s.stride_px = g.stride(l);
            push(s, nullptr);
        }
        return true;
    }
    bool head_close(Head &hd)
    {
        lane = 0;
        if (!p->fused_head && !p->f32) push(hd.h3s, nullptr);
        return err.empty();
    }

    bool build()
    {
        const rva_yolov8_desc &d = p->d;
        const int c3 = g.c[3], c4 = g.c[4], c5 = g.c[5];
        auto block = [&](int i, const Src &src, View dst, int l, const char *what) {
            const bool shortcut = i < 4;
            return c2f(dst.ch / 2, shortcut ? d.depth_backbone[i] : d.depth_head, src, dst, l, what,
                       [&](View x, View y) { return pair(x, y, shortcut, l, what); });
        };
        static const char *const backbone_names[7] = {"b2", "b3", "b4", "b5", "b6", "b7", "b8"}, *const up_names[4] = {"h16", "h18", "h19", "h21"};
        View cat12 = buf(4, c5 + c4), cat15 = buf(3, c4 + c3), cat18 = buf(4, c3 + c4), cat21 = buf(5, c4 + c5);
        View p4 = cat12.sub(c5, c4), p3 = cat15.sub(c4, c3), n4 = cat18.sub(c3, c4), p5 = cat21.sub(c4, c5), n3 = buf(3, c3), x1, feats[3];
        if (!stem(3, "b0", "b1", &x1) || !backbone(block, x1, buf(2, g.c[2]), p3, p4, p5, backbone_names) ||
            !top_down(block, p5, cat12, cat15, n4, n3, "h12", "h15") || !bottom_up(block, n3, cat18, cat21, feats, up_names)) return false;
        Head hd;
        if (!head_open(hd)) return false;
        const int cb = hd.cb, cc = hd.cc;
        const rva_conv_weights *cls[3][3];
        for (int l = 0; l < 3; ++l) {
            cls[l][0] = take(g.c[3 + l], hd.cc_real, 3, 1, "detect.cls.0"); cls[l][1] = take(hd.cc_real, hd.cc_real, 3, 1, "detect.cls.1");
            cls[l][2] = take(hd.cc_real, d.nc, 1, 1, "detect.cls.2");
            if (!cls[l][0] || !cls[l][1] || !cls[l][2]) return false;
            cls[l][0] = padded(cls[l][0], g.c[3 + l], cc); cls[l][1] = padded(cls[l][1], cc, cc); cls[l][2] = padded(cls[l][2], cc, hd.ncp);
        }
        if (!all_taken()) return false;
        for (int l = 0; l < 3; ++l) {
            lane = ((p->fused_head || p->f32) && l < 2) ? l + 1 : 0;
            if (lane) p->fork_step[lane] = fork_at[l];
            View first = buf(3 + l, cb + cc), b2 = buf(3 + l, cb), k2 = buf(3 + l, cc);
            const rva_conv_weights *sib[2] = {hd.box[l][0], cls[l][0]};
            if (!conv(sib, 2, feats[l], first, 3 + l, 1)) return false;
            if (!conv1(hd.box[l][1], first.sub(0, cb), b2, 3 + l, 1) || !head_last(hd, 3 + l, 1, hd.box[l][2], b2)) return false;
            if (!conv1(cls[l][1], first.sub(cb, cc), k2, 3 + l, 1) || !head_last(hd, 3 + l, 2, cls[l][2], k2)) return false;
        }
        return head_close(hd);
    }

    bool build_v5(const float *anchors)
    {
        const rva_yolov8_desc &d = p->d;
        const int c3w = g.c[3], c4 = g.c[4], c5 = g.c[5];
        if (c3w % 64 || c4 % 64 || c5 % 64) return fail("YOLOv5 plan: c3, c4 and c5 must be multiples of 64 (the upsample + concat and head kernels)");
        auto block = [&](int i, const Src &src, View dst, int l, const char *what) {
            return c3(i < 4 ? d.depth_backbone[i] : d.depth_head, i < 4, src, dst, l, what);
        };
        static const char *const backbone_names[7] = {"b2", "b3", "b4", "b5", "b6", "b7", "b8"}, *const up_names[4] = {"h18", "h20", "h21", "h23"};
        View cat20 = buf(4, 2 * c3w), cat23 = buf(5, 2 * c4), t14 = cat20.sub(c3w, c3w), t10 = cat23.sub(c4, c4);
        View p3 = buf(3, c3w), p4 = buf(4, c4), p5 = buf(5, c5), n4 = buf(4, c4), n3 = buf(3, c3w), x1, feats[3];
        if (!stem(6, "b0", "b1", &x1) || !backbone(block, x1, buf(2, g.c[2]), p3, p4, p5, backbone_names)) return false;
        if (!conv1(take(c5, c4, 1, 1, "h10"), p5, t10, 5, 1) || !block(4, Src(t10, p4), n4, 4, "h13") ||
            !conv1(take(c4, c3w, 1, 1, "h14"), n4, t14, 4, 1) || !block(5, Src(t14, p3), n3, 3, "h17")) return false;
        if (!bottom_up(block, n3, cat20, cat23, feats, up_names)) return false;
        const int co_real = 3 * (5 + d.nc), co = (co_real + 7) / 8 * 8;
        p->A = 3 * g.a0(6);
        const void *danc = nullptr;
        if (!upload(anchors, sizeof(float) * 18, &danc)) return false;
        for (int l = 3; l <= 5; ++l) {
            const rva_conv_weights *hc = padded(take(g.c[l], co_real, 1, 1, "detect.m"), g.c[l], co);
            Step s{}; s.kind = K_HEAD5;
            if (!hc || !pack(&hc, 1, s)) return false;
            const View &f = feats[l - 3];
            s.in = f.ptr(); s.ldi = f.ld; s.H = g.h[l]; s.W = g.w[l]; s.a0 = 3 * g.a0(l); s.stride_px = g.stride(l);
            s.b2 = (const float *)danc + 6 * (l - 3);
            push(s, "head5:%d->%d k1s1 %dx%d", s.Cin, s.Cout, s.H, s.W);
        }
        return all_taken() && err.empty();
    }

    bool build_11(const rva_yolo11_desc &e)
    {
        const int c3w = g.c[3], c4 = g.c[4], c5 = g.c[5];
        auto block = [&](int i, const Src &src, View dst, int l, const char *what) {
            const int c = i < 2 ? dst.ch / 4 : dst.ch / 2;
            const bool shortcut = i < 4;
            if (e.repeats[i] < 1 || c % 16) return fail("a C3k2 block needs at least one inner block and an inner width that is a multiple of 16");
            return c2f(c, e.repeats[i], src, dst, l, what, [&](View x, View y) {
                return e.c3k[i] ? c3(2, shortcut, x, y, l, what, 3) : bottleneck(x, y, c / 2, shortcut, l, what);
            });
        };
        static const char *const backbone_names[7] = {"2", "3", "4", "5", "6", "7", "8"}, *const up_names[4] = {"17", "19", "20", "22"};
        View cat13 = buf(4, c5 + c4), cat16 = buf(3, c4 + c4), cat19 = buf(4, c3w + c4), cat22 = buf(5, c4 + c5);
        View p4 = cat13.sub(c5, c4), p3 = cat16.sub(c4, c4), n4 = cat19.sub(c3w, c4), p5 = cat22.sub(c4, c5), t5 = buf(5, c5), n3 = buf(3, c3w), x1, feats[3];
        if (!stem(3, "0", "1", &x1) || !backbone(block, x1, buf(2, c3w), p3, p4, t5, backbone_names) || !c2psa(e.psa_blocks, e.psa_heads, t5, p5) ||
            !top_down(block, p5, cat13, cat16, n4, n3, "13", "16") || !bottom_up(block, n3, cat19, cat22, feats, up_names)) return false;
        Head hd;
        if (!head_open(hd)) return false;
        const int cb = hd.cb, cr = hd.cc_real, cc = hd.cc;
        const rva_conv_weights *cls[3][5];
        for (int l = 0; l < 3; ++l) {
            const int ch = g.c[3 + l];
            cls[l][0] = take(1, ch, 3, 1, "detect.cls.0.0"); cls[l][1] = take(ch, cr, 1, 1, "detect.cls.0.1");
            cls[l][2] = take(1, cr, 3, 1, "detect.cls.1.0"); cls[l][3] = take(cr, cr, 1, 1, "detect.cls.1.1");
            cls[l][4] = take(cr, p->d.nc, 1, 1, "detect.cls.2");
            for (int i = 0; i < 5; ++i)
                if (!cls[l][i]) return false;
            cls[l][1] = padded(cls[l][1], ch, cc); cls[l][2] = padded(cls[l][2], 1, cc); cls[l][3] = padded(cls[l][3], cc, cc);
            cls[l][4] = padded(cls[l][4], cc, hd.ncp);
        }
        if (!all_taken()) return false;
        for (int l = 0; l < 3; ++l) {
            const int L = 3 + l;
            const View &f = feats[l];
            View bb1 = buf(L, cb), bb2 = buf(L, cb), d1 = buf(L, f.ch), k1 = buf(L, cc), d2 = buf(L, cc), k2 = buf(L, cc);
            if (!conv1(hd.box[l][0], f, bb1, L, 1) || !conv1(hd.box[l][1], bb1, bb2, L, 1)) return false;
            if (!dwconv(cls[l][0], 0, f, d1, L, 1) || !conv1(cls[l][1], d1, k1, L, 1) || !dwconv(cls[l][2], 0, k1, d2, L, 1) ||
                !conv1(cls[l][3], d2, k2, L, 1)) return false;
            if (!head_last(hd, L, 1, hd.box[l][2], bb2) || !head_last(hd, L, 2, cls[l][4], k2)) return false;
        }
        return head_close(hd);
    }
};

bool step_takes_rows(const Step &s, int variant)
{
    if (s.kind == K_STEM2 || s.kind == K_STEM6) return true;
    return s.kind == K_CONV && rva_conv_variant_rows(variant, s.Cin, s.k, s.stride);
}

int launch_step(rva_yolov8_plan *p, const Step &s, int variant, const void *input, void *output, int n, rva_stream_t st, bool win)
{
    rva_ctx *c = p->ctx;
    if (win && (s.y0 > 0 || s.y1 < s.Ho) && step_takes_rows(s, variant)) {
        if (s.kind == K_STEM2) return rva_stem2_f16_rows(c, input, s.w, s.b, s.w2, s.b2, s.out, s.ldo, n, s.H, s.W, s.y0, s.y1, st);
        if (s.kind == K_STEM6) return rva_stem6_conv_f16_rows(c, input, s.w, s.b, s.out, s.ldo, n, s.H, s.W, s.Cout, s.y0, s.y1, st);
        return rva_conv2d_nhwc_f16_sel(c, s.in, s.ldi, s.w, s.b, s.out, s.ldo, s.res, s.ldr, n, p->B, s.H, s.W, s.Cin, s.Cout, s.k, s.stride, s.act,
                                       variant, s.y0, s.y1, st);
    }
    float *boxes = p->box32 && output ? (float *)((char *)output + p->box_off) : nullptr;
    switch (s.kind) {
    case K_CONV: return rva_conv2d_nhwc_f16_sel(c, s.in, s.ldi, s.w, s.b, s.out, s.ldo, s.res, s.ldr, n, p->B, s.H, s.W, s.Cin, s.Cout, s.k, s.stride, s.act, variant,
                                                0, -1, st);
    case K_UPCAT: return rva_conv1x1_upcat_f16(c, s.in, s.ldi, s.c_in, s.in2, s.ldi2, s.c_in2, s.w, s.b, s.out, s.ldo, n, s.H, s.W, s.Cout, s.act, variant, st);
    case K_HEAD: return rva_conv1x1_head_nc_f16(c, s.in, s.ldi, s.w, s.b, n, s.H, s.W, s.Cin, s.Cout, s.mode, output, s.mode == 1 ? boxes : nullptr, p->nc,
                                                p->A, s.a0, s.stride_px, variant, st);
    case K_PAIR32: return rva_c2f_pair32_f16(c, s.in, s.ldi, s.w, s.b, s.w2, s.b2, s.out, s.ldo, n, s.H, s.W, st);
    case K_STEM2: return rva_stem2_f16(c, input, s.w, s.b, s.w2, s.b2, s.out, s.ldo, n, s.H, s.W, st);
    case K_STEM: return rva_stem_conv_f16(c, input, s.w, s.b, s.out, s.ldo, n, s.H, s.W, s.Cout, st);
    case K_SPPF3: return rva_sppf_pool3_nhwc_f16(c, s.in, s.ldi, s.out, s.out2, s.out3, s.ldo, n, s.H, s.W, s.Cin, st);
    case K_POOL5: return rva_maxpool5_nhwc_f16(c, s.in, s.ldi, s.out, s.ldo, n, s.H, s.W, s.Cin, st);
    case K_UP2: return rva_upsample2x_nhwc_f16(c, s.in, s.ldi, s.out, s.ldo, n, s.H, s.W, s.Cin, st);
    case K_HEAD3: return rva_yolo_head3_nc_f16(c, s.hb, s.hldb, s.hk, s.hldc, output, boxes, n, s.hh, s.hw, p->nc, p->A, s.hs, st);
    case K_CONV_F32: return rva_conv2d_nhwc_f32_v(c, s.in, s.ldi, s.w, s.b, s.out, s.ldo, s.res, s.ldr, n, s.H, s.W, s.Cin, s.Cout, s.k, s.stride, s.act, variant, st);
    case K_STEM_F32: return rva_stem_conv_f32(c, input, s.w, s.b, s.out, s.ldo, n, s.H, s.W, s.Cout, st);
    case K_POOL5_F32: return rva_maxpool5_nhwc_f32(c, s.in, s.ldi, s.out, s.ldo, n, s.H, s.W, s.Cin, st);
    case K_UP2_F32: return rva_upsample2x_nhwc_f32(c, s.in, s.ldi, s.out, s.ldo, n, s.H, s.W, s.Cin, st);
    case K_STEM6: return rva_stem6_conv_f16(c, input, s.w, s.b, s.out, s.ldo, n, s.H, s.W, s.Cout, st);
    case K_HEAD5: return rva_conv1x1_head5_f16(c, s.in, s.ldi, s.w, s.b, n, s.H, s.W, s.Cin, p->nc, s.b2, output, boxes, p->A, s.a0, s.stride_px, variant, st);
    case K_HEAD_F32: return rva_yolo_head_f32(c, s.in, s.ldi, s.in2, s.ldi2, output, n, s.H, s.W, p->nc, p->A, s.a0, s.stride_px, st);
    case K_DWCONV: return rva_dwconv3x3_nhwc_f16(c, s.in, s.ldi, s.w, s.b, s.out, s.ldo, s.res, s.ldr, n, s.H, s.W, s.Cin, s.act, st);
    case K_ATTN: return rva_psa_attention_f16(c, s.in, s.ldi, s.out, s.ldo, n, s.H * s.W, s.mode, st);
    }
    return RVA_ERR_ARG;
}

bool variant_fits(const Step &s, int variant)
{
    if (s.kind == K_CONV) return variant >= 0;
    if (s.kind == K_CONV_F32) return variant >= 0 && variant <= rva_conv_f32_num_variants();
    return variant == 0 || rva_conv_variant_is_gather64(variant);
}

int out_rows(int H, int k, int stride) { return (H + 2 * (k / 2) - k) / stride + 1; }

void propagate_rows(rva_yolov8_plan *p)
{
    struct Slice { const char *lo, *hi; int H, y0, y1; };
    std::vector<Slice> written;
    const int es = p->f32 ? 4 : 2;
    const bool off = p->f32 || (p->rows_top <= 0 && p->rows_bottom >= p->H);
    auto read = [&](const void *ptr, int ch, int H, int *lo, int *hi) {
        const char *a = (const char *)ptr, *b = a + (size_t)ch * es;
        long covered = 0;
        int y0 = H, y1 = 0;
        for (const Slice &w : written) {
            const char *l = w.lo > a ? w.lo : a, *h = w.hi < b ? w.hi : b;
            if (l >= h) continue;
            if (w.H != H) return false;
            covered += h - l;
            if (w.y0 < y0) y0 = w.y0;
            if (w.y1 > y1) y1 = w.y1;
        }
        if (covered != b - a || y0 >= y1) return false;
        *lo = y0; *hi = y1;
        return true;
    };
    auto through = [](int k, int stride, int H, int *lo, int *hi) {
        int32_t a = 0, b = 0;
        (void)rva_conv_rows_through(k, stride, H, *lo, *hi, &a, &b);
        *lo = a; *hi = b;
        return out_rows(H, k, stride);
    };
    p->windowed = false;
    for (Step &s : p->steps) {
        int lo = 0, hi = 0, Ho = s.H;
        bool known = false;
        switch (s.kind) {
        case K_STEM2: case K_STEM:
            lo = p->rows_top; hi = p->rows_bottom; known = true;
            Ho = through(3, 2, s.H, &lo, &hi);
            if (s.kind == K_STEM2) Ho = through(3, 2, Ho, &lo, &hi);
            break;
        case K_STEM6: {
            int32_t a = 0, b = 0;
            (void)rva_conv_rows_through_pad(6, 2, 2, s.H, p->rows_top, p->rows_bottom, &a, &b);
            lo = a; hi = b; known = true; Ho = s.H / 2;
            break;
        }
        case K_CONV:
            known = read(s.in, s.c_real, s.H, &lo, &hi);
            Ho = out_rows(s.H, s.k, s.stride);
            if (known) {
                (void)through(s.k, s.stride, s.H, &lo, &hi);
                int rl = 0, rh = 0;
                if (s.res) {
                    known = read(s.res, s.Cout, Ho, &rl, &rh);
                    if (rl < lo) lo = rl;
                    if (rh > hi) hi = rh;
                }
            }
            break;
        case K_PAIR32:
            known = read(s.in, 32, s.H, &lo, &hi);
            if (known) { (void)through(3, 1, s.H, &lo, &hi); (void)through(3, 1, s.H, &lo, &hi); }
            break;
        case K_UPCAT: {
            int l2 = 0, h2 = 0;
            known = read(s.in, s.c_in, s.H / 2, &lo, &hi) && read(s.in2, s.c_in2, s.H, &l2, &h2);
            lo = 2 * lo < l2 ? 2 * lo : l2;
            hi = 2 * hi > h2 ? 2 * hi : h2;
            break;
        }
        default: break;
        }
        s.Ho = Ho;
        if (off || !known || lo >= hi) { lo = 0; hi = Ho; }
        s.y0 = lo; s.y1 = hi;
        if (lo > 0 || hi < Ho) p->windowed = true;
        if (s.kind == K_STEM2 || s.kind == K_STEM || s.kind == K_STEM6 || s.kind == K_CONV || s.kind == K_PAIR32 || s.kind == K_UPCAT) {
            const int ch = s.kind == K_STEM2 ? 64 : s.kind == K_PAIR32 ? 32 : s.Cout;
            written.push_back(Slice{(const char *)s.out, (const char *)s.out + (size_t)ch * es, Ho, lo, hi});
        }
    }
    for (Tunable &t : p->tunables) {
        const Step &s = p->steps[t.step];
        t.desc = t.base;
        if (s.y0 > 0 || s.y1 < s.Ho) {
            char w[32];
            snprintf(w, sizeof w, " r[%d,%d)", s.y0, s.y1);
            t.desc += w;
        }
    }
    p->primed = 0;
}

bool stream_is_capturing(rva_stream_t stream)
{
    hipStreamCaptureStatus cs = hipStreamCaptureStatusNone;
    if (hipStreamIsCapturing((hipStream_t)stream, &cs) != hipSuccess) { (void)hipGetLastError(); return false; }
    return cs != hipStreamCaptureStatusNone;
}

int run_steps(rva_yolov8_plan *p, const void *input, void *output, int n, int first, int last, rva_stream_t stream, bool win)
{
    for (int i = first; i < last; ++i) {
        const Step &s = p->steps[i];
        const int rc = launch_step(p, s, s.variant, input, output, n, stream, win);
        if (rc != RVA_OK) return rc;
    }
    return RVA_OK;
}

int check_run(rva_yolov8_plan *p, const void *input, void *output, int n)
{
    if (!p || !input || !output) return RVA_ERR_ARG;
    if (n <= 0 || n > p->B) return rva_fail(p->ctx, RVA_ERR_ARG, "rva_yolov8_plan_run: n = %d is not 1 .. %d, the plan's capacity", n, p->B);
    if (((uintptr_t)input | (uintptr_t)output) % 16) return rva_fail(p->ctx, RVA_ERR_ARG, "rva_yolov8_plan_run: input and output must be 16-byte aligned");
    return RVA_OK;
}

void note_complete_run(rva_yolov8_plan *p, int n, bool win, rva_stream_t stream)
{
    if (!win && !stream_is_capturing(stream)) p->primed = n;
}

template <typename D>
rva_yolov8_desc internal_desc(const D &e)
{
    rva_yolov8_desc d{};
    d.batch = e.batch; d.height = e.height; d.width = e.width; d.nc = e.nc; d.reg_max = 16; d.n_convs = e.n_convs; d.flags = e.flags;
    memcpy(d.widths, e.widths, sizeof d.widths);
    return d;
}

struct PlanDeleter { void operator()(rva_yolov8_plan *p) const { rva_yolov8_plan_destroy(p); } };

template <typename Refuse, typename Build>
int create_plan(rva_ctx *ctx, const char *who, const char *also, const rva_yolov8_desc &d, int head_rows, const rva_conv_weights *convs,
                rva_yolov8_plan **out, Refuse refuse, Build build)
{
    *out = nullptr;
    if (d.batch <= 0 || d.height <= 0 || d.width <= 0 || d.height % 32 || d.width % 32 || d.nc < 1 || d.nc > 1024 || d.reg_max != 16 || d.n_convs <= 0)
        return rva_fail(ctx, RVA_ERR_ARG, "%s: batch > 0, height and width multiples of 32, 1 <= nc <= 1024%s", who, also);
    for (int i = 0; i < 5; ++i)
        if (d.widths[i] <= 0 || d.widths[i] % 8) return rva_fail(ctx, RVA_ERR_ARG, "%s: channel widths must be multiples of 8", who);
    if (const int rc = refuse(); rc != RVA_OK) return rc;
    RVA_HIP(ctx, hipSetDevice(ctx->device));
    std::unique_ptr<rva_yolov8_plan, PlanDeleter> p(new rva_yolov8_plan());
    p->ctx = ctx; p->d = d; p->B = d.batch; p->H = d.height; p->W = d.width; p->nc = d.nc;
    p->head_rows = head_rows;
    p->f32 = (d.flags & RVA_PLAN_F32) != 0;
    p->box32 = (d.flags & RVA_PLAN_BOX_F32) != 0;
    Builder b(p.get(), convs);
    if (!build(b)) return rva_fail(ctx, b.hip_failed ? RVA_ERR_HIP : RVA_ERR_ARG, "%s: %s", who, b.err.c_str());
    for (int l = 1; l <= 2; ++l)
        if (p->fork_step[l] >= 0) {
            RVA_HIP(ctx, hipEventCreateWithFlags(&p->fork_ev[l], hipEventDisableTiming));
            RVA_HIP(ctx, hipEventCreateWithFlags(&p->join_ev[l], hipEventDisableTiming));
        }
    RVA_HIP(ctx, hipDeviceSynchronize());
    if (p->box32) p->box_off = ((size_t)p->B * p->head_rows * p->A * 2 + 255) / 256 * 256;
    p->rows_top = 0; p->rows_bottom = p->H;
    propagate_rows(p.get());
    *out = p.release();
    return RVA_OK;
}

}

extern "C" {

int rva_yolov8_plan_create(rva_ctx *ctx, const rva_yolov8_desc *desc, const rva_conv_weights *convs, rva_yolov8_plan **out)
{
    if (!ctx || !desc || !convs || !out) return RVA_ERR_ARG;
    const char *who = "rva_yolov8_plan_create";
    return create_plan(ctx, who, ", reg_max 16", *desc, 4 + desc->nc, convs, out, [&] {
        if ((desc->flags & RVA_PLAN_F32) && (desc->flags & RVA_PLAN_BOX_F32))
            return rva_fail(ctx, RVA_ERR_ARG, "%s: RVA_PLAN_BOX_F32 belongs to fp16 plans (the output of an RVA_PLAN_F32 plan is fp32 already)", who);
        return (int)RVA_OK;
    }, [](Builder &b) { return b.build(); });
}

int rva_yolov5_plan_create(rva_ctx *ctx, const rva_yolov5_desc *desc, const rva_conv_weights *convs, rva_yolov8_plan **out)
{
    if (!ctx || !desc || !convs || !out) return RVA_ERR_ARG;
    const char *who = "rva_yolov5_plan_create";
    rva_yolov8_desc d = internal_desc(*desc);
    memcpy(d.depth_backbone, desc->depth_backbone, sizeof d.depth_backbone);
    d.depth_head = desc->depth_head;
    return create_plan(ctx, who, "", d, 5 + desc->nc, convs, out, [&] {
        if (desc->flags & RVA_PLAN_F32) return rva_fail(ctx, RVA_ERR_ARG, "%s: there is no fp32 YOLOv5 plan (RVA_PLAN_F32); build the fp16 plan", who);
        for (int i = 0; i < 18; ++i)
            if (!(desc->anchors[i] > 0.f) || !(desc->anchors[i] < 65504.f)) return rva_fail(ctx, RVA_ERR_ARG, "%s: anchors must be positive pixel sizes", who);
// ... 58 lines not shown
    if (s.tunable >= 0) { snprintf(buf, (size_t)len, "%s", p->tunables[s.tunable].desc.c_str()); return RVA_OK; }
    switch (s.kind) {
    case K_ATTN: snprintf(buf, (size_t)len, "attention heads %d tokens %d", s.mode, s.H * s.W); break;
    case K_DWCONV: snprintf(buf, (size_t)len, "dwconv3x3 %d act%d%s %dx%d", s.Cin, s.act, s.res ? " +res" : "", s.H, s.W); break;
    case K_STEM2: snprintf(buf, (size_t)len, "stem2 3->32->64 %dx%d", s.H, s.W); break;
    case K_STEM: case K_STEM_F32: snprintf(buf, (size_t)len, "stem 3->%d k3s2 %dx%d", s.Cout, s.H, s.W); break;
    case K_STEM6: snprintf(buf, (size_t)len, "stem6 3->%d k6s2 %dx%d", s.Cout, s.H, s.W); break;
    case K_PAIR32: snprintf(buf, (size_t)len, "pair32 %dx%d", s.H, s.W); break;
    case K_SPPF3: snprintf(buf, (size_t)len, "sppf pool3 %d %dx%d", s.Cin, s.H, s.W); break;
    case K_POOL5: case K_POOL5_F32: snprintf(buf, (size_t)len, "maxpool5 %d %dx%d", s.Cin, s.H, s.W); break;
    case K_UP2: case K_UP2_F32: snprintf(buf, (size_t)len, "upsample2x %d %dx%d", s.Cin, s.H, s.W); break;
    case K_HEAD3: snprintf(buf, (size_t)len, "head3 decode"); break;
    case K_HEAD_F32: snprintf(buf, (size_t)len, "head decode %dx%d", s.H, s.W); break;
    default: snprintf(buf, (size_t)len, "step kind %d", (int)s.kind); break;
    }
    return RVA_OK;
}

int rva_yolov8_plan_set_variant(rva_yolov8_plan *p, int index, int variant)
{
    if (!p || index < 0 || index >= (int)p->tunables.size()) return RVA_ERR_ARG;
    Step &s = p->steps[p->tunables[index].step];
    if (!variant_fits(s, variant) || variant > rva_conv_num_variants()) return rva_fail(p->ctx, RVA_ERR_ARG, "rva_yolov8_plan_set_variant: variant %d does not exist for this layer", variant);
    p->primed = 0;
    s.variant = variant;
    return RVA_OK;
}

int rva_yolov8_plan_get_variant(const rva_yolov8_plan *p, int index)
{
    if (!p || index < 0 || index >= (int)p->tunables.size()) return -1;
    return p->steps[p->tunables[index].step].variant;
}

int rva_yolov8_plan_launch_tunable(rva_yolov8_plan *p, int index, int variant, void *output, rva_stream_t stream)
{
    if (!p || index < 0 || index >= (int)p->tunables.size()) return RVA_ERR_ARG;
    const Step &s = p->steps[p->tunables[index].step];
    if (!variant_fits(s, variant)) return RVA_ERR_ARG;
    if ((s.kind == K_HEAD || s.kind == K_HEAD5) && !output) return RVA_ERR_ARG;
    return launch_step(p, s, variant, nullptr, output, p->B, stream, true);
}

int rva_yolov8_plan_run_range_n(rva_yolov8_plan *p, const void *input, void *output, int n, int first, int last, rva_stream_t stream)
{
    if (const int rc = check_run(p, input, output, n); rc != RVA_OK) return rc;
    if (first < 0 || last > (int)p->steps.size() || first > last) return RVA_ERR_ARG;
    return run_steps(p, input, output, n, first, last, stream, n <= p->primed);
}

int rva_yolov8_plan_run_range(rva_yolov8_plan *p, const void *input, void *output, int first, int last, rva_stream_t stream)
{
    return p ? rva_yolov8_plan_run_range_n(p, input, output, p->B, first, last, stream) : RVA_ERR_ARG;
}

int rva_yolov8_plan_run_n(rva_yolov8_plan *p, const void *input, void *output, int n, rva_stream_t stream)
{
    if (const int rc = check_run(p, input, output, n); rc != RVA_OK) return rc;
    const bool win = n <= p->primed;
    const int rc = run_steps(p, input, output, n, 0, (int)p->steps.size(), stream, win);
    if (rc == RVA_OK) note_complete_run(p, n, win, stream);
    return rc;
}

int rva_yolov8_plan_run(rva_yolov8_plan *p, const void *input, void *output, rva_stream_t stream)
{
    return p ? rva_yolov8_plan_run_n(p, input, output, p->B, stream) : RVA_ERR_ARG;
}

int rva_yolov8_plan_primed_images(const rva_yolov8_plan *p) { return p ? p->primed : 0; }

int rva_yolov8_plan_set_static_rows(rva_yolov8_plan *p, int top, int bottom)
{
    if (!p) return RVA_ERR_ARG;
    if (top < 0 || bottom > p->H || top >= bottom)
        return rva_fail(p->ctx, RVA_ERR_ARG, "rva_yolov8_plan_set_static_rows: [%d, %d) is not a window of %d rows", top, bottom, p->H);
    const char *e = getenv("RVA_PLAN_NO_STATIC_ROWS");
    if (e && e[0] == '1') return RVA_OK;
    p->rows_top = top; p->rows_bottom = bottom;
    propagate_rows(p);
    return RVA_OK;
}

int rva_yolov8_plan_step_rows(const rva_yolov8_plan *p, int step, int32_t *y0, int32_t *y1)
{
    if (!p || step < 0 || step >= (int)p->steps.size()) return RVA_ERR_ARG;
    if (y0) *y0 = p->steps[step].y0;
    if (y1) *y1 = p->steps[step].y1;
    return RVA_OK;
}

int rva_conv_rows_through(int k, int stride, int H_in, int lo, int hi, int32_t *out_lo, int32_t *out_hi)
{
    if ((k != 1 && k != 3) || (stride != 1 && stride != 2)) return RVA_ERR_ARG;
    return rva_conv_rows_through_pad(k, stride, k / 2, H_in, lo, hi, out_lo, out_hi);
}

int rva_conv_rows_through_pad(int k, int stride, int pad, int H_in, int lo, int hi, int32_t *out_lo, int32_t *out_hi)
{
    if (k < 1 || stride < 1 || pad < 0 || pad >= k || H_in <= 0 || lo < 0 || hi > H_in || lo >= hi || !out_lo || !out_hi) return RVA_ERR_ARG;
    if (H_in + 2 * pad < k) return RVA_ERR_ARG;
    const int Ho = (H_in + 2 * pad - k) / stride + 1;
    int a = lo + pad - (k - 1), b = hi - 1 + pad;
    a = a <= 0 ? 0 : (a + stride - 1) / stride;
    b = b / stride + 1;
    if (b > Ho) b = Ho;
    if (a > b) a = b;
    *out_lo = a; *out_hi = b;
    return RVA_OK;
}

int rva_yolov8_plan_run_lanes(rva_yolov8_plan *p, const void *input, void *output, rva_stream_t stream, rva_stream_t side1, rva_stream_t side2)
{
    return p ? rva_yolov8_plan_run_lanes_n(p, input, output, p->B, stream, side1, side2) : RVA_ERR_ARG;
}

int rva_yolov8_plan_run_lanes_n(rva_yolov8_plan *p, const void *input, void *output, int n, rva_stream_t stream, rva_stream_t side1, rva_stream_t side2)
{
    if (const int rc = check_run(p, input, output, n); rc != RVA_OK) return rc;
    if (!side1 || !side2 || p->fork_step[1] < 0) return rva_yolov8_plan_run_n(p, input, output, n, stream);
    hipStream_t lanes[3] = {(hipStream_t)stream, (hipStream_t)side1, (hipStream_t)side2};
    bool started[3] = {true, false, false};
    const bool win = n <= p->primed;
    for (int i = 0; i < (int)p->steps.size(); ++i) {
        for (int l = 1; l <= 2; ++l)
            if (p->fork_step[l] == i) RVA_HIP(p->ctx, hipEventRecord(p->fork_ev[l], lanes[0]));
        const Step &s = p->steps[i];
        if (s.lane && !started[s.lane]) {
            RVA_HIP(p->ctx, hipStreamWaitEvent(lanes[s.lane], p->fork_ev[s.lane], 0));
            started[s.lane] = true;
        }
        const int rc = launch_step(p, s, s.variant, input, output, n, (rva_stream_t)lanes[s.lane], win);
        if (rc != RVA_OK) return rc;
    }
    for (int l = 1; l <= 2; ++l)
        if (started[l]) {
            RVA_HIP(p->ctx, hipEventRecord(p->join_ev[l], lanes[l]));
            RVA_HIP(p->ctx, hipStreamWaitEvent(lanes[0], p->join_ev[l], 0));
        }
    note_complete_run(p, n, win, stream);
    return RVA_OK;
}

}
```

### realtime_video_analytics_32streams_amd/detector.py

```python
from __future__ import annotations

import abc
import logging
from dataclasses import dataclass
from typing import Iterable, List, Optional, Sequence

import numpy as np
import torch

from . import _native as N
from . import ops
from .config import HIP_BACKENDS, TEMPORAL_MODELS, DetectorConfig
from .video_stream import FramePacket
from .yolov8 import build_detector_net, variant_from_path

LOGGER = logging.getLogger(__name__)


@dataclass(slots=True)
class Detection:

    stream_name: str
    frame_id: int
    class_id: int
# ... 4 lines not shown
class BaseDetector(abc.ABC):

    def __init__(self, config: DetectorConfig):
        self.config = config

    @abc.abstractmethod
    def predict(self, packet: FramePacket) -> List[Detection]:
        raise NotImplementedError


def filter_detections(detections: Iterable[Detection], min_confidence: float) -> List[Detection]:
    return [d for d in detections if d.confidence >= min_confidence]


def create_detector(config: DetectorConfig) -> BaseDetector:
    backend = config.backend.lower()
    model_type = config.model_type.lower()
    if backend in HIP_BACKENDS:
        if model_type in TEMPORAL_MODELS:
            from .temporal import HipCNN3DDetector, HipCNNLSTMDetector, HipConvGRUDetector
            if model_type == "cnn_lstm":
                return HipCNNLSTMDetector(config)
            if model_type == "conv_gru":
                return HipConvGRUDetector(config)
            return HipCNN3DDetector(config)
        if model_type == "resnet":
            from .classify import HipResNetDetector
            return HipResNetDetector(config)
        if model_type in ("yolov5", "yolov8"):
            return HipYoloDetector(config)
        raise ValueError(f"Model type '{model_type}' not supported with backend '{config.backend}'")
    if backend in ("ultralytics", "tensorrt", "onnx", "onnxruntime", "openvino", "rknn", "rk3588"):
        raise RuntimeError(
            f"Detector backend '{config.backend}' belongs to the reference implementation and its runtime is not "
            "part of this library. Select backend 'hip' to run on MI355X.")
    raise ValueError(f"Unsupported detector backend '{config.backend}'")


def detector_architecture(model_type: str, model_path: str, net=None, state_dict=None) -> str:
    from .yolo11 import Yolo11, is_11_state_dict, variant_from_path_11
    from .yolov5 import YoloV5, is_v5_state_dict, variant_from_path_v5
    if net is not None:
        return "yolo11" if isinstance(net, Yolo11) else "yolov5" if isinstance(net, YoloV5) else "yolov8"
    if _is_file(model_path):
        if state_dict is None:
            state_dict = torch.load(model_path, map_location="cpu", weights_only=True)
        return "yolo11" if is_11_state_dict(state_dict) else "yolov5" if is_v5_state_dict(state_dict) else "yolov8"
    if variant_from_path_11(model_path) is not None:
        return "yolo11"
    if str(model_type).lower() == "yolov5" and variant_from_path_v5(model_path) is not None:
        return "yolov5"
    return "yolov8"


def v5_scale_of(model_path: str, state_dict=None) -> str:
    from .yolov5 import variant_from_path_v5
    for key in ("b0.conv.weight", "model.0.conv.weight", "0.conv.weight") if state_dict is not None else ():
        w = state_dict.get(key)
        if w is not None:
            s = {16: "n", 32: "s", 48: "m", 64: "l", 80: "x"}.get(int(w.shape[0]))
            if s:
                return s
    return variant_from_path_v5(model_path) or "n"


def select_yolo_engine(arch: str, half: bool, hip_engine: str = "auto") -> str:
    if half:
        return "fused"
    if hip_engine in ("plan", "native"):
        if arch in ("yolov5", "yolo11"):
            name = "YOLOv5" if arch == "yolov5" else "YOLO11"
            raise ValueError(f"hip_engine: {hip_engine} with half: false needs an fp32 {name} plan, which does not exist; the "
                             f"hand-written {name} plan is fp16: set `half: true` (or `hip_engine: auto` for fp32 through PyTorch-ROCm)")
        return "fused-f32"
    return "torch-fp32"


class HipYoloDetector(BaseDetector):

    def __init__(self, config: DetectorConfig, infer_fn=None, net: Optional[torch.nn.Module] = None,
                 seed: int = 0, device: Optional[int] = None):
        super().__init__(config)
        self._plans = {}
        self.ctx = ops.context(device)
        self.device = torch.device("cuda", self.ctx.device)
        if config.input_size:
            self.input_hw = (int(config.input_size[0]), int(config.input_size[1]))
        else:
            self.input_hw = (640, 640)
        self.half = bool(config.half)
        sd = None
        if infer_fn is None and net is None and _is_file(config.model_path):
            sd = torch.load(config.model_path, map_location="cpu", weights_only=True)
        self.arch = "yolov8" if infer_fn is not None else detector_architecture(config.model_type, config.model_path, net, sd)
        self.engine = select_yolo_engine(self.arch, self.half, getattr(config, "hip_engine", "auto"))
        self._infer_fn = infer_fn
        self.box_rows = getattr(config, "hip_box_rows", "fp16") if (self.engine == "fused" and infer_fn is None) else "fp16"
        cap = int(getattr(config, "hip_plan_capacity", 0) or 0)
        self.plan_capacity = cap if (infer_fn is None and self.engine in ("fused", "fused-f32")) else 0
        self._over_capacity_warned = False
        self.net = None
        if infer_fn is None:
            if net is None and self.arch == "yolo11":
                from .yolo11 import build_detector_net_11, scale_of_11
                scale = scale_of_11(config.model_path, sd)
                net = build_detector_net_11(scale, seed=seed, weights=config.model_path)
                LOGGER.info("hip detector: YOLO11%s, %s weights", scale,
                            "local state-dict" if sd is not None else "seeded random (no weights offline)")
            elif net is None and self.arch == "yolov5":
                from .yolov5 import build_detector_net_v5
                scale = v5_scale_of(config.model_path, sd)
                net = build_detector_net_v5(scale, seed=seed, weights=config.model_path)
                LOGGER.info("hip detector: YOLOv5%s, %s weights", scale,
                            "local state-dict" if sd is not None else "seeded random (no weights offline)")
            elif net is None:
                scale = variant_from_path(config.model_path)
                net = build_detector_net(scale, seed=seed, weights=config.model_path)
                LOGGER.info("hip detector: YOLOv8%s, %s weights", scale,
                            "local state-dict" if _is_file(config.model_path) else "seeded random (no weights offline)")
            if self.engine == "torch-fp32":
                LOGGER.warning("hip detector: half=false -> fp32 network through PyTorch-ROCm (MIOpen); the hand-written fp16 "
                               "MFMA plan runs with `half: true`")
            net = net.fuse().to(self.device)
            net = net.half() if self.half else net.float()
            self.net = net.to(memory_format=torch.channels_last)
        self._post_bufs: dict = {}
        self._in_bufs: dict = {}
        self._in_border: dict = {}
        self._rows: dict = {}
        self._rows_told: dict = {}
        self._post: Optional[ops.PostBuffers] = None
        self._in: Optional[torch.Tensor] = None
        self._slot = 0
        if config.warmup and self.net is not None:
            with torch.inference_mode():
                self._infer(torch.zeros((1, 3, *self.input_hw), device=self.device,
                                        dtype=torch.float16 if self.half else torch.float32))

    def _images(self, batch: int) -> int:
        cap = self.plan_capacity
        if cap <= 0 or batch == cap:
            return batch
        if batch > cap:
            if not self._over_capacity_warned:
                self._over_capacity_warned = True
                LOGGER.warning("hip detector: a group of %d frames exceeds hip_plan_capacity=%d: it gets a plan of its own size, "
                               "built now", batch, cap)
            return batch
        return cap

    def _buf_key(self, batch: int):
        m = self._images(batch)
        return m if self._slot == 0 else (m, self._slot)

    def input_tensor(self, batch: int) -> torch.Tensor:
        n, m = self._buf_key(batch), self._images(batch)
        t = self._in_bufs.get(n)
        if t is None:
            dt = torch.float16 if self.half else torch.float32
            t = self._in_bufs[n] = torch.empty((m, 3, *self.input_hw), dtype=dt, device=self.device)
        return t if m == batch else t[:batch]

    def _preprocess(self, frames: Sequence) -> tuple[torch.Tensor, N.Letterbox]:
        n = self._buf_key(len(frames))
        self._in = self.input_tensor(len(frames))
        f0 = frames[0]
        if isinstance(f0, ops.Nv12Surface):
            key = (f0.width, f0.height) if not any(f.mask is not None for f in frames) else None
            have, bordered = self._in_border.get(n, (None, 0))
            steady = key is not None and have == key and len(frames) <= bordered
            res = ops.preprocess_nv12(frames, self.input_hw, self.half, out=self._in, ctx=self.ctx, content_only=steady)
            if not steady:
                self._in_border[n] = (key, len(frames))
                lb = res[1]
                self._note_rows(n, (int(lb.pad_top), int(lb.pad_top) + int(lb.new_h)) if key is not None else (0, self.input_hw[0]))
            return res
        dev = []
        for f in frames:
            t = torch.from_numpy(np.ascontiguousarray(f)) if isinstance(f, np.ndarray) else f
            dev.append(t.to(self.device, non_blocking=True).contiguous())
        self._in_border[n] = (None, 0)
        self._note_rows(n, (0, self.input_hw[0]))
        return ops.preprocess_bgr(dev, self.input_hw, self.half, out=self._in, ctx=self.ctx)

    def _note_rows(self, n, rows) -> None:
        rows = (max(rows[0], 0), min(rows[1], self.input_hw[0]))
        self._rows[n] = rows
        self._rows_told[n] = False

    def invalidate_engine(self) -> None:
        self._plans.clear()
        self._rows_told.clear()

    def plan_for(self, tensor: torch.Tensor):
        batch = int(tensor.shape[0])
        shape = (self._images(batch), int(tensor.shape[2]), int(tensor.shape[3]))
        key = shape if self._slot == 0 else shape + (self._slot,)
        plan = self._plans.get(key)
        if plan is None:
            from .engine import FusedYolo11, FusedYoloV5, FusedYoloV8
            plan_cls = {"yolov5": FusedYoloV5, "yolo11": FusedYolo11}.get(self.arch, FusedYoloV8)
            first = self._plans.get(shape) if self._slot else None
            n = shape[0] if self._slot == 0 else (shape[0], self._slot)
            rows = first.static_rows if first is not None else self._rows.get(n)
            plan = self._plans[key] = plan_cls(self.net, shape[0], shape[1:], device=self.device, ctx=self.ctx,
                                               autotune=first is None, tune_overlap=getattr(self, "tune_overlap", 1),
                                               precision="fp32" if self.engine == "fused-f32" else "fp16", box_rows=self.box_rows,
                                               static_rows=rows if self.engine == "fused" else None)
            if first is not None:
                plan.copy_tuning(first)
        plan.n = batch
        return plan

    def rows_pending(self, batch: int) -> bool:
        return not self._rows_told.get(self._buf_key(batch), True)

    def _tell_rows(self, plan, tensor: torch.Tensor) -> None:
        n = self._buf_key(int(tensor.shape[0]))
        own = self._in_bufs.get(n)
        if own is None or own.data_ptr() != tensor.data_ptr() or n not in self._rows:
            if plan.static_rows != (0, plan.H):
                plan.set_static_rows(0, plan.H)
                if n in self._rows:
                    self._rows_told[n] = False
            return
        if self._rows_told.get(n, True):
            return
        plan.set_static_rows(*self._rows[n])
        self._rows_told[n] = True

    def _infer(self, tensor: torch.Tensor):
        if self._infer_fn is not None:
            return self._infer_fn(tensor)
        if self.half:
            if tensor.dtype != torch.float16:
                raise TypeError("half detector: the fused plan takes the fp16 tensor K1 writes")
            plan = self.plan_for(tensor)
            if not torch.cuda.is_current_stream_capturing():
                self._tell_rows(plan, tensor)
            plan(tensor.contiguous())
            return plan.result()
        if self.engine == "fused-f32":
            if tensor.dtype != torch.float32:
                raise TypeError("fp32 plan: takes the fp32 tensor K1 writes for half=false")
            return self.plan_for(tensor)(tensor.contiguous())
        return self.net(tensor.float().contiguous(memory_format=torch.channels_last))

    def _postprocess_device(self, raw, metas: Sequence[N.Letterbox]) -> ops.PostBuffers:
        boxes = None
        if isinstance(raw, ops.SplitHead):
            raw, boxes = raw
        raw = raw.contiguous()
        B = raw.shape[0]
        A = raw.shape[2] if raw.shape[1] < raw.shape[2] else raw.shape[1]
        self._post = self._post_bufs.get((B, A))
        if self._post is None:
            self._post = self._post_bufs[(B, A)] = ops.PostBuffers.allocate(B, A, raw.device)
        return ops.postprocess(raw, self.config.confidence_threshold, self.config.iou_threshold, self.config.classes,
                               metas, max_det=A, out=self._post, ctx=self.ctx, boxes=boxes)

    def stage_pre(self, packets: Sequence[FramePacket]):
        return self._preprocess([p.frame for p in packets])

    def stage_net(self, pre):
        return self._infer(pre[0])

    def stage_post(self, raw, pre) -> ops.PostBuffers:
        return self._postprocess_device(raw, [pre[1]])

    @staticmethod
    def geometry_key(frame) -> tuple:
        if isinstance(frame, ops.Nv12Surface):
            return (int(frame.width), int(frame.height), "nv12")
        return (int(frame.shape[1]), int(frame.shape[0]), "bgr")

    def predict_batch_device(self, packets: Sequence[FramePacket]) -> ops.PostBuffers:
        if len({self.geometry_key(p.frame) for p in packets}) != 1:
            raise ValueError("predict_batch_device needs one frame geometry per call; use predict_batch for mixed sizes")
        with torch.inference_mode():
            tensor, meta = self._preprocess([p.frame for p in packets])
            raw = self._infer(tensor)
            return self._postprocess_device(raw, [meta])

    def predict_batch(self, packets: Sequence[FramePacket]) -> List[List[Detection]]:
        out: List[Optional[List[Detection]]] = [None] * len(packets)
        groups = {}
        for i, p in enumerate(packets):
            groups.setdefault(self.geometry_key(p.frame), []).append(i)
        for idxs in groups.values():
            res = self.predict_batch_device([packets[i] for i in idxs]).to_host()
            for i, r in zip(idxs, res):
                p = packets[i]
                out[i] = [Detection(stream_name=p.stream.name, frame_id=p.frame_id, class_id=int(r["cls"][k]),
                                    confidence=float(r["conf"][k]),
                                    bbox_xyxy=tuple(float(v) for v in r["boxes"][k])) for k in range(r["n"])]
        return out

    def predict(self, packet: FramePacket) -> List[Detection]:
        return self.predict_batch([packet])[0]


def _is_file(p: str) -> bool:
    from pathlib import Path
    return bool(p) and Path(p).is_file()
```

### realtime_video_analytics_32streams_amd/engine.py

```python
from __future__ import annotations

import ctypes as C
import hashlib
import json
import os
from pathlib import Path
from typing import Optional, Tuple

import numpy as np
import torch

from . import _native as N
from . import ops
from .yolov8 import C2f, ConvBnAct, YoloV8


_LIB_DIGEST: Optional[str] = None


def _lib_digest() -> str:
    global _LIB_DIGEST
    if _LIB_DIGEST is None:
        _LIB_DIGEST = hashlib.sha256(N.LIB_PATH.read_bytes()).hexdigest()
    return _LIB_DIGEST


def _tuning_dir():
    d = os.environ.get("RVA_TUNE_CACHE_DIR")
    return Path(d) if d else Path(os.environ.get("XDG_CACHE_HOME", str(Path.home() / ".cache"))) / "rva_amd" / "autotune"


def module_order_convs(net: YoloV8) -> list:
    def c2f(m: C2f):
        out = [m.cv1, m.cv2]
        for b in m.m:
            out += [b.cv1, b.cv2]
        return out
    mods = [net.b0, net.b1, *c2f(net.b2), net.b3, *c2f(net.b4), net.b5, *c2f(net.b6), net.b7, *c2f(net.b8), net.b9.cv1, net.b9.cv2,
            *c2f(net.h12), *c2f(net.h15), net.h16, *c2f(net.h18), net.h19, *c2f(net.h21)]
    for branch in (net.detect.box, net.detect.cls):
        for seq in branch:
            mods += [seq[0], seq[1], seq[2]]
    return [m.conv if isinstance(m, ConvBnAct) else m for m in mods]


class _VariantCell:

    __slots__ = ("eng", "idx")

    def __init__(self, eng, idx):
        self.eng, self.idx = eng, idx

    def __getitem__(self, key):
        assert key == "variant"
        return int(self.eng.L.rva_yolov8_plan_get_variant(self.eng.handle, self.idx))

    def __setitem__(self, key, value):
        assert key == "variant"
        self.eng.ctx.check(self.eng.L.rva_yolov8_plan_set_variant(self.eng.handle, self.idx, int(value)), "rva_yolov8_plan_set_variant")


class FusedYoloV8:
    HEAD_ROWS_EXTRA = 4
    ARCH_KEY = b""

    def __init__(self, net: YoloV8, batch: int, hw: Tuple[int, int] = (640, 640), device: Optional[torch.device] = None,
                 ctx: Optional[N.Context] = None, autotune: bool = True, tune_overlap: int = 1, precision: str = "fp16",
                 box_rows: str = "fp16", static_rows: Optional[Tuple[int, int]] = None):
        if precision not in ("fp16", "fp32"):
            raise ValueError(f"precision must be 'fp16' or 'fp32', not {precision!r}")
        if box_rows not in ("fp16", "fp32"):
            raise ValueError(f"box_rows must be 'fp16' or 'fp32', not {box_rows!r}")
        if box_rows == "fp32" and precision == "fp32":
            raise ValueError("box_rows='fp32' belongs to the fp16 plan: the output of precision='fp32' is fp32 already")
        self.box_rows = box_rows
        self.precision = precision
        self.f32 = precision == "fp32"
        self.tune_overlap = int(tune_overlap)
        self.ctx = ctx or ops.context()
        self.dev = device or torch.device("cuda", self.ctx.device)
        self.B, self.H, self.W = batch, hw[0], hw[1]
        self.n = batch
        assert hw[0] % 32 == 0 and hw[1] % 32 == 0
        net = net.fuse()
        self.nc = net.nc
        self.L = N.lib()
        convs = self._module_order(net)
        keep, arr = [], (N.ConvWeights * len(convs))()
        for i, c in enumerate(convs):
            w = np.ascontiguousarray(c.weight.detach().float().cpu().numpy())
            b = None if c.bias is None else np.ascontiguousarray(c.bias.detach().float().cpu().numpy())
            keep += [w, b]
            arr[i].weight = w.ctypes.data_as(C.POINTER(C.c_float))
            arr[i].bias = b.ctypes.data_as(C.POINTER(C.c_float)) if b is not None else None
            arr[i].cout, arr[i].cin, arr[i].k, arr[i].stride = int(w.shape[0]), int(w.shape[1]), int(w.shape[2]), int(c.stride[0])
        d, create = self._descriptor(net, batch, hw, len(convs))
        d.flags = (N.RVA_PLAN_NO_STEM2 if os.environ.get("RVA_NO_STEM2", "0") == "1" else 0) | \
                  (N.RVA_PLAN_NO_CIN_PAD if os.environ.get("RVA_NO_CIN_PAD", "0") == "1" else 0) | \
                  (0 if self._use_pair32() else N.RVA_PLAN_NO_PAIR32) | \
                  (N.RVA_PLAN_F32 if self.f32 else 0) | (N.RVA_PLAN_BOX_F32 if box_rows == "fp32" else 0)
        h = C.c_void_p()
        with torch.cuda.device(self.dev):
            self.ctx.check(getattr(self.L, create)(self.ctx.handle, C.byref(d), arr, C.byref(h)), create)
        self.handle = h
        del keep
        self.static_rows = (0, self.H)
        self.rows_epoch = 0
        if static_rows is not None and tuple(static_rows) != (0, self.H) and os.environ.get("RVA_PLAN_NO_STATIC_ROWS") != "1":
            self.ctx.check(self.L.rva_yolov8_plan_set_static_rows(h, int(static_rows[0]), int(static_rows[1])), "rva_yolov8_plan_set_static_rows")
            self.static_rows = (int(static_rows[0]), int(static_rows[1]))
        info = [C.c_int32() for _ in range(5)]
        self.ctx.check(self.L.rva_yolov8_plan_info(h, *[C.byref(v) for v in info]), "rva_yolov8_plan_info")
        self.A, rows, self._n_steps, n_tun, self.quiet_step = (int(v.value) for v in info)
        assert rows == self.HEAD_ROWS_EXTRA + self.nc
        self.dtype = torch.float32 if self.f32 else torch.float16
        self.boxes32: Optional[torch.Tensor] = None
        self._boxes = {}
        if box_rows == "fp32":
            total, off = C.c_int64(), C.c_int64()
            self.ctx.check(self.L.rva_yolov8_plan_output_layout(h, C.byref(total), C.byref(off)), "rva_yolov8_plan_output_layout")
            self._out_layout = (int(total.value), int(off.value))
            self.out, self.boxes32 = self._alloc_split()
            self._boxes[0] = self.boxes32
        else:
            self.out = torch.empty((batch, rows, self.A), dtype=self.dtype, device=self.dev)
        self._outs = {0: self.out}
        self.fused_stem = isinstance(d, (N.YoloV8Desc, N.Yolo11Desc)) and not self.f32 and not (d.flags & N.RVA_PLAN_NO_STEM2) and tuple(d.widths[:2]) == (32, 64)
        self._n_tunable = n_tun
        self._read_tunables()
        self._side = None
        self._forks = bool(self.fused_head_lanes())
        self.concurrent_heads = os.environ.get("RVA_SERIAL_HEADS") != "1"
        if autotune:
            self.autotune()

    @staticmethod
    def _module_order(net) -> list:
        return module_order_convs(net)

    @staticmethod
    def _descriptor(net, batch: int, hw: Tuple[int, int], n_convs: int):
        d = N.YoloV8Desc()
        d.batch, d.height, d.width = batch, hw[0], hw[1]
        d.widths[:] = [net.b0.conv.out_channels, net.b1.conv.out_channels, net.b3.conv.out_channels, net.b5.conv.out_channels,
                       net.b7.conv.out_channels]
        d.depth_backbone[:] = [len(net.b2.m), len(net.b4.m), len(net.b6.m), len(net.b8.m)]
        d.depth_head = len(net.h12.m)
        assert len(net.h15.m) == len(net.h18.m) == len(net.h21.m) == d.depth_head
        d.nc, d.reg_max, d.n_convs = net.nc, net.detect.reg_max, n_convs
        return d, "rva_yolov8_plan_create"

    def _read_tunables(self) -> None:
        self._tunable = []
        buf = C.create_string_buffer(96)
        for i in range(self._n_tunable):
            self.ctx.check(self.L.rva_yolov8_plan_tunable_desc(self.handle, i, buf, 96), "rva_yolov8_plan_tunable_desc")

            def launch(stream, variant, i=i):
                return self.L.rva_yolov8_plan_launch_tunable(self.handle, i, variant, C.c_void_p(self.out.data_ptr()), stream)
            self._tunable.append((launch, _VariantCell(self, i), buf.value.decode()))

    def set_static_rows(self, top: int, bottom: int) -> None:
        self.ctx.check(self.L.rva_yolov8_plan_set_static_rows(self.handle, int(top), int(bottom)), "rva_yolov8_plan_set_static_rows")
        if os.environ.get("RVA_PLAN_NO_STATIC_ROWS") == "1":
            return
        self.static_rows = (int(top), int(bottom))
        self.rows_epoch += 1
        self._read_tunables()

    @property
    def primed_images(self) -> int:
        return int(self.L.rva_yolov8_plan_primed_images(self.handle))

    @property
    def primed(self) -> bool:
        return self.primed_images >= self.n

    def step_rows(self, step: int) -> Tuple[int, int]:
        y0, y1 = C.c_int32(), C.c_int32()
        self.ctx.check(self.L.rva_yolov8_plan_step_rows(self.handle, int(step), C.byref(y0), C.byref(y1)), "rva_yolov8_plan_step_rows")
        return int(y0.value), int(y1.value)

    def step_desc(self, step: int) -> str:
        buf = C.create_string_buffer(96)
        self.ctx.check(self.L.rva_yolov8_plan_step_desc(self.handle, int(step), buf, 96), "rva_yolov8_plan_step_desc")
        return buf.value.decode()

    def _alloc_split(self) -> Tuple[torch.Tensor, torch.Tensor]:
        total, off = self._out_layout
        rows = self.HEAD_ROWS_EXTRA + self.nc
        buf = torch.empty((total,), dtype=torch.uint8, device=self.dev)
        head = buf[:self.B * rows * self.A * 2].view(torch.float16).view(self.B, rows, self.A)
        boxes = buf[off:off + self.B * 4 * self.A * 4].view(torch.float32).view(self.B, 4, self.A)
        return head, boxes

    def fused_head_lanes(self) -> bool:
        return self.f32 or any(d.startswith("head1:") for _, _, d in self._tunable)

    def __del__(self):
        try:
            if getattr(self, "handle", None):
                self.L.rva_yolov8_plan_destroy(self.handle)
                self.handle = None
        except Exception:
            pass

    def _tuning_key(self) -> str:
        h = hashlib.sha256()
        h.update(torch.cuda.get_device_name(self.dev).encode())
        h.update(_lib_digest().encode())
        h.update(repr((self.B, self.H, self.W, [d for _, _, d in self._tunable])).encode())
        h.update(b"per-layer times; in-plan pass opt-in, three overlapping passes")
        skip, no_stem2, no_cin_pad = (os.environ.get(k, "") for k in ("RVA_SKIP_VARIANTS", "RVA_NO_STEM2", "RVA_NO_CIN_PAD"))
        h.update(repr([skip, "", "", "", "", no_stem2, "", no_cin_pad]).encode())
        h.update(repr(int(os.environ.get("RVA_TUNE_LAYER_OVERLAP", getattr(self, "tune_overlap", 1)))).encode())
        if getattr(self, "f32", False):
            h.update(b"precision fp32")
        if self.ARCH_KEY:
            h.update(self.ARCH_KEY)
        return h.hexdigest()[:24]

    def _load_tuning(self) -> bool:
        f = _tuning_dir() / f"{self._tuning_key()}.json"
        try:
            rec = json.loads(f.read_text())
            picks = rec["variants"]
            if len(picks) != len(self._tunable) or any(d != pd for (_, _, d), (pd, _) in zip(self._tunable, picks)):
                return False
        except (OSError, ValueError, KeyError, TypeError):
            return False
        try:
            for (_, state, _), (_, v) in zip(self._tunable, picks):
                state["variant"] = int(v)
        except RuntimeError:
            for _, state, _ in self._tunable:
                state["variant"] = 0
            return False
        self.tuning = [tuple(t) for t in rec.get("tuning", [])]
        self.tuning_source = str(f)
        return True

    def _store_tuning(self) -> None:
        d = _tuning_dir()
        try:
            d.mkdir(parents=True, exist_ok=True)
            tmp = d / f".{self._tuning_key()}.{os.getpid()}.tmp"
            tmp.write_text(json.dumps({"device": torch.cuda.get_device_name(self.dev), "batch": self.B, "hw": [self.H, self.W],
                                       "variants": [[desc, st["variant"]] for _, st, desc in self._tunable],
                                       "tuning": [list(t) for t in self.tuning]}))
            os.replace(tmp, d / f"{self._tuning_key()}.json")
        except OSError:
# ... 210 lines not shown
```

Measured before the change: 23890.

## Gate YOLOv8 box branch tail on class-score threshold bitmap

The classification head now writes a per-anchor bitmap of cells whose objectness or top class score passes the confidence threshold. The last box-branch conv layers (3x3 conv plus 1x1 conv and DFL decode) are skipped in the normal plan and replaced by a sparse tail kernel that computes boxes only for gated anchors using MFMA. This removes most box-branch compute in the pipelined stage path, at the cost of atomics, a gate clear and a compacting kernel. Box rows for anchors below threshold are left stale or unwritten, which postprocess must ignore.

```diff
diff --git a/include/rva.h b/include/rva.h
--- a/include/rva.h
+++ b/include/rva.h
@@ -253,6 +253,9 @@
 int rva_yolov8_plan_run_range_n(rva_yolov8_plan *plan, const void *input, void *output, int n, int first, int last, rva_stream_t stream);
 int rva_yolov8_plan_primed_images(const rva_yolov8_plan *plan);
 int rva_yolov8_plan_step_rows(const rva_yolov8_plan *plan, int step, int32_t *y0, int32_t *y1);
+int rva_yolov8_plan_set_box_gate(rva_yolov8_plan *plan, double conf);
+int rva_yolov8_plan_box_gate(const rva_yolov8_plan *plan);
+int rva_box_gate_threshold_f16(double conf);
 int rva_yolov8_plan_step_desc(const rva_yolov8_plan *plan, int step, char *buf, int len);
 
 typedef struct rva_yolov5_desc {
diff --git a/realtime_video_analytics_32streams_amd/_native.py b/realtime_video_analytics_32streams_amd/_native.py
--- a/realtime_video_analytics_32streams_amd/_native.py
+++ b/realtime_video_analytics_32streams_amd/_native.py
@@ -11,7 +11,7 @@
 ROOT = PKG.parent
 CSRC = PKG / "csrc"
 LIB_PATH = Path(os.environ["RVA_LIB_PATH"]) if os.environ.get("RVA_LIB_PATH") else PKG / "librva.so"
-SOURCES = ["rva_ctx.hip", "rva_preprocess.hip", "rva_postprocess.hip", "rva_tracker.hip", "rva_conv.hip", "rva_stem.hip", "rva_yolo_ops.hip", "rva_conv_f32.hip", "rva_attn.hip", "rva_plan.hip", "rva_clip.hip",
+SOURCES = ["rva_ctx.hip", "rva_preprocess.hip", "rva_postprocess.hip", "rva_tracker.hip", "rva_conv.hip", "rva_stem.hip", "rva_yolo_ops.hip", "rva_conv_f32.hip", "rva_attn.hip", "rva_box_tail.hip", "rva_plan.hip", "rva_clip.hip",
            "rva_clip3d.hip", "rva_clip_f16.hip", "rva_resnet.hip", "rva_resnet_f16.hip", "rva_gates.hip", "rva_decode.hip", "rva_preview.hip", "rva_jpeg.hip", "rva_jpeg_dec.hip"]
 HIPCC_FLAGS = ["--offload-arch=gfx950", "-O3", "-fPIC", "-shared", "-std=c++17", "-ffp-contract=off",
                "-Wall", "-Wno-unused-function"]
@@ -281,6 +281,9 @@
         "rva_yolov8_plan_run_lanes_n": (C.c_int, [_P, _P, _P, C.c_int, _P, _P, _P]),
         "rva_yolov8_plan_run_range_n": (C.c_int, [_P, _P, _P, C.c_int, C.c_int, C.c_int, _P]),
         "rva_yolov8_plan_primed_images": (C.c_int, [_P]),
+        "rva_yolov8_plan_set_box_gate": (C.c_int, [_P, C.c_double]),
+        "rva_yolov8_plan_box_gate": (C.c_int, [_P]),
+        "rva_box_gate_threshold_f16": (C.c_int, [C.c_double]),
         "rva_yolov5_plan_create": (C.c_int, [_P, C.POINTER(YoloV5Desc), C.POINTER(ConvWeights), C.POINTER(_P)]),
         "rva_stem6_conv_f16": (C.c_int, [_P, _P, _P, _P, _P, C.c_int, C.c_int, C.c_int, C.c_int, C.c_int, _P]),
         "rva_stem6_conv_f16_rows": (C.c_int, [_P, _P, _P, _P, _P, C.c_int, C.c_int, C.c_int, C.c_int, C.c_int, C.c_int, C.c_int, _P]),
@@ -391,6 +394,7 @@
     "rva_resnetx_f16_plan_create", "rva_resnetx_f16_plan_destroy", "rva_resnetx_f16_plan_info", "rva_resnetx_f16_plan_run",
     "rva_resnetx_f16_plan_run_post", "rva_resnetx_f16_plan_stage",
     "rva_jpeg_dec_probe", "rva_jpeg_dec_create", "rva_jpeg_dec_destroy", "rva_jpeg_dec_decode", "rva_jpeg_dec_status", "rva_jpeg_dec_times",
+    "rva_yolov8_plan_set_box_gate", "rva_yolov8_plan_box_gate", "rva_box_gate_threshold_f16",
 ]
 
 
diff --git a/realtime_video_analytics_32streams_amd/csrc/rva_box_tail.hip b/realtime_video_analytics_32streams_amd/csrc/rva_box_tail.hip
--- /dev/null
+++ b/realtime_video_analytics_32streams_amd/csrc/rva_box_tail.hip
@@ -0,0 +1,139 @@
+#include "rva_conv_dev.h"
+
+namespace {
+
+struct TailLevel {
+    const __half *in; int ld;
+    int H, W, a0, blk0;
+    float stride;
+    const __half *w1; const float *b1;
+    const __half *w2; const float *b2;
+};
+
+struct TailArgs {
+    TailLevel lv[3];
+    const uint32_t *gate; int plane;
+    __half *out;
+    float *box32;
+    int nc, A, nwords, bpi;
+};
+
+__device__ __forceinline__ uint2 tail_round4(const f4 acc, const float4 bv, bool act)
+{
+    float v0 = acc[0] + bv.x, v1 = acc[1] + bv.y, v2 = acc[2] + bv.z, v3 = acc[3] + bv.w;
+    if (act) { v0 = silu_f(v0); v1 = silu_f(v1); v2 = silu_f(v2); v3 = silu_f(v3); }
+    __half2 lo = __floats2half2_rn(v0, v1), hi = __floats2half2_rn(v2, v3);
+    uint2 pk;
+    pk.x = *reinterpret_cast<uint32_t *>(&lo);
+    pk.y = *reinterpret_cast<uint32_t *>(&hi);
+    return pk;
+}
+
+__global__ void __launch_bounds__(256) k_box_tail(TailArgs a)
+{
+    constexpr int TROW = 64 + 8;
+    __shared__ int list[256];
+    __shared__ int wcnt[4];
+    __shared__ __attribute__((aligned(16))) __half t1[16 * TROW], t2[16 * TROW];
+
+    const int tid = threadIdx.x, lane = tid & 63, wv = tid >> 6;
+    const int b = blockIdx.x / a.bpi, r = blockIdx.x - b * a.bpi;
+    const int l = r >= a.lv[2].blk0 ? 2 : r >= a.lv[1].blk0 ? 1 : 0;
+    const TailLevel L = l == 2 ? a.lv[2] : l == 1 ? a.lv[1] : a.lv[0];
+    const int HW = L.H * L.W;
+
+    const int cell = (r - L.blk0) * 256 + tid, at = L.a0 + cell;
+    bool set = false;
+    if (cell < HW && at < a.A) {
+        const uint32_t *w = a.gate + (size_t)b * a.nwords + (at >> 5);
+        uint32_t m = w[0];
+        if (a.nc > 1) m &= w[a.plane];
+        set = (m >> (at & 31)) & 1u;
+    }
+    const unsigned long long bal = __ballot(set);
+    if (lane == 0) wcnt[wv] = __popcll(bal);
+    __syncthreads();
+    int base = 0, total = 0;
+#pragma unroll
+    for (int w = 0; w < 4; ++w) {
+        const int c = wcnt[w];
+        if (w < wv) base += c;
+        total += c;
+    }
+    if (total == 0) return;
+    if (set) list[base + __popcll(bal & ((1ull << lane) - 1ull))] = cell;
+    __syncthreads();
+
+    const int px = lane & 15, kq = lane >> 4;
+    const __half *img = L.in + (size_t)b * HW * L.ld;
+    const __half *w1row = L.w1 + (size_t)(16 * wv + px) * (9 * 64) + kq * 8;
+    const __half *w2row = L.w2 + (size_t)(16 * wv + px) * 64 + kq * 8;
+    const float4 bv1 = *reinterpret_cast<const float4 *>(L.b1 + 16 * wv + kq * 4);
+    const float4 bv2 = *reinterpret_cast<const float4 *>(L.b2 + 16 * wv + kq * 4);
+    const h8 hz = {0, 0, 0, 0, 0, 0, 0, 0};
+
+    for (int g0 = 0; g0 < total; g0 += 16) {
+        const bool valid = g0 + px < total;
+        const int c = valid ? list[g0 + px] : 0;
+        const int y = c / L.W, x = c - y * L.W;
+        f4 acc = {0.f, 0.f, 0.f, 0.f};
+#pragma unroll
+        for (int dy = 0; dy < 3; ++dy)
+#pragma unroll
+            for (int ch = 0; ch < 2; ++ch)
+#pragma unroll
+                for (int dx = 0; dx < 3; ++dx) {
+                    const int iy = y + dy - 1, ix = x + dx - 1;
+                    const bool ok = valid && (unsigned)iy < (unsigned)L.H && (unsigned)ix < (unsigned)L.W;
+                    const h8 bf = ok ? *reinterpret_cast<const h8 *>(img + ((size_t)iy * L.W + ix) * L.ld + ch * 32 + kq * 8) : hz;
+                    const h8 af = *reinterpret_cast<const h8 *>(w1row + (dy * 3 + dx) * 64 + ch * 32);
+                    acc = __builtin_amdgcn_mfma_f32_16x16x32_f16(af, bf, acc, 0, 0, 0);
+                }
+        *reinterpret_cast<uint2 *>(t1 + px * TROW + 16 * wv + kq * 4) = tail_round4(acc, bv1, true);
+        __syncthreads();
+        f4 acc2 = {0.f, 0.f, 0.f, 0.f};
+#pragma unroll
+        for (int ks = 0; ks < 2; ++ks) {
+            const h8 bf = *reinterpret_cast<const h8 *>(t1 + px * TROW + ks * 32 + kq * 8);
+            const h8 af = *reinterpret_cast<const h8 *>(w2row + ks * 32);
+            acc2 = __builtin_amdgcn_mfma_f32_16x16x32_f16(af, bf, acc2, 0, 0, 0);
+        }
+        *reinterpret_cast<uint2 *>(t2 + px * TROW + 16 * wv + kq * 4) = tail_round4(acc2, bv2, false);
+        __syncthreads();
+        if (tid < 16 && g0 + tid < total) {
+            const int ci = list[g0 + tid];
+            const size_t o = (size_t)L.a0 + ci;
+            head_box_decode(t2 + tid * TROW, ci, L.W, L.stride, a.out + (size_t)b * (4 + a.nc) * a.A + o,
+                            a.box32 ? a.box32 + (size_t)b * 4 * a.A + o : nullptr, (size_t)a.A);
+        }
+    }
+}
+
+}
+
+int rva_box_tail_f16(rva_ctx *ctx, const rva_box_tail_level *levels, const uint32_t *gate, int gate_plane, void *out, float *boxes32,
+                     int n, int nc, int anchors_total, rva_stream_t stream_)
+{
+    if (!ctx) return RVA_ERR_ARG;
+    if (!levels || !gate || gate_plane < n * ((anchors_total + 31) / 32) || !out || n <= 0 || nc < 1 || anchors_total <= 0 || (uintptr_t)gate % 4 || (uintptr_t)out % 2 || (uintptr_t)boxes32 % 4)
+        return rva_fail(ctx, RVA_ERR_ARG, "rva_box_tail_f16: bad arguments");
+    TailArgs a{};
+    int blocks = 0;
+    for (int l = 0; l < 3; ++l) {
+        const rva_box_tail_level &s = levels[l];
+        if (!s.first || !s.w1 || !s.b1 || !s.w2 || !s.b2 || s.H <= 0 || s.W <= 0 || s.H > 2000 || s.W > 2000 || s.ld < 64 || s.ld % 8 || s.a0 < 0 ||
+            (long)s.a0 + (long)s.H * s.W > anchors_total || ((uintptr_t)s.first | (uintptr_t)s.w1 | (uintptr_t)s.w2 | (uintptr_t)s.b1 | (uintptr_t)s.b2) % 16)
+            return rva_fail(ctx, RVA_ERR_ARG, "rva_box_tail_f16: level %d: 64 box channels in rows of ld %% 8 == 0 halfs, 16-byte aligned tensors, the level "
+                                              "inside the anchor range", l);
+        TailLevel &d = a.lv[l];
+        d.in = (const __half *)s.first; d.ld = s.ld; d.H = s.H; d.W = s.W; d.a0 = s.a0; d.blk0 = blocks; d.stride = s.stride_px;
+        d.w1 = (const __half *)s.w1; d.b1 = s.b1; d.w2 = (const __half *)s.w2; d.b2 = s.b2;
+        blocks += rva_ceil_div(s.H * s.W, 256);
+    }
+    if ((long)n * blocks >= (1l << 31)) return rva_fail(ctx, RVA_ERR_ARG, "rva_box_tail_f16: too many workgroups");
+    a.gate = gate; a.plane = gate_plane; a.out = (__half *)out; a.box32 = boxes32; a.nc = nc; a.A = anchors_total; a.nwords = (anchors_total + 31) / 32; a.bpi = blocks;
+    hipLaunchKernelGGL(k_box_tail, dim3((unsigned)(n * blocks)), dim3(256), 0, (hipStream_t)stream_, a);
+    const hipError_t e = hipGetLastError();
+    if (e != hipSuccess) return rva_fail(ctx, RVA_ERR_HIP, "rva_box_tail_f16: launch failed: %s", hipGetErrorString(e));
+    return RVA_OK;
+}
diff --git a/realtime_video_analytics_32streams_amd/csrc/rva_conv.hip b/realtime_video_analytics_32streams_amd/csrc/rva_conv.hip
--- a/realtime_video_analytics_32streams_amd/csrc/rva_conv.hip
+++ b/realtime_video_analytics_32streams_amd/csrc/rva_conv.hip
@@ -10,6 +10,7 @@
     union {
         const __half *res;
         float *hbox;
+        uint32_t *hgate;
     };
     int ldr;
     int CoutPad;
@@ -18,7 +19,14 @@
         const __half *in2;
         const float *hanc;
     };
-    int ldi2, c_split;
+    union {
+        int ldi2;
+        int hgate_plane;
+    };
+    union {
+        int c_split;
+        float hgate_thr;
+    };
     int H, W, Cin, CinPad, Ho, Wo, Cout, stride, M, act, n_tiles, m_tiles;
     int wy0, wrows;
 };
@@ -1493,44 +1501,23 @@
             __half *o = a.hout + (size_t)b * (4 + a.hnc) * a.hA + a.ha0 + i;
             const __half *row = stage + (size_t)r * SROW;
             if (a.hmode == 1) {
-                float d[4];
-#pragma unroll
-                for (int sd = 0; sd < 4; ++sd) {
-                    float v[16], mx = -1e30f;
-                    const uint4 q0 = *reinterpret_cast<const uint4 *>(row + sd * 16), q1 = *reinterpret_cast<const uint4 *>(row + sd * 16 + 8);
-                    const __half2 *h0 = reinterpret_cast<const __half2 *>(&q0), *h1 = reinterpret_cast<const __half2 *>(&q1);
-#pragma unroll
-                    for (int t = 0; t < 4; ++t) {
-                        float2 f = __half22float2(h0[t]); v[2 * t] = f.x; v[2 * t + 1] = f.y;
-                        f = __half22float2(h1[t]); v[8 + 2 * t] = f.x; v[9 + 2 * t] = f.y;
-                    }
-#pragma unroll
-                    for (int t = 0; t < 16; ++t) mx = fmaxf(mx, v[t]);
-                    float se = 0.f, sw = 0.f;
-#pragma unroll
-                    for (int t = 0; t < 16; ++t) { const float e = __expf(v[t] - mx); se += e; sw += e * (float)t; }
-                    d[sd] = sw / se;
-                }
-                const float ax = (float)(i % a.hW) + 0.5f, ay = (float)(i / a.hW) + 0.5f;
-                const float x1 = ax - d[0], y1 = ay - d[1], x2 = ax + d[2], y2 = ay + d[3];
-                o[0] = __float2half_rn((x1 + x2) * 0.5f * a.hstride);
-                o[(size_t)a.hA] = __float2half_rn((y1 + y2) * 0.5f * a.hstride);
-                o[(size_t)2 * a.hA] = __float2half_rn((x2 - x1) * a.hstride);
-                o[(size_t)3 * a.hA] = __float2half_rn((y2 - y1) * a.hstride);
-                if (a.hbox) {
-                    float *o32 = a.hbox + (size_t)b * 4 * a.hA + a.ha0 + i;
-                    o32[0] = (x1 + x2) * 0.5f * a.hstride;
-                    o32[(size_t)a.hA] = (y1 + y2) * 0.5f * a.hstride;
-                    o32[(size_t)2 * a.hA] = (x2 - x1) * a.hstride;
-                    o32[(size_t)3 * a.hA] = (y2 - y1) * a.hstride;
-                }
+                head_box_decode(row, i, a.hW, a.hstride, o, a.hbox ? a.hbox + (size_t)b * 4 * a.hA + a.ha0 + i : nullptr, (size_t)a.hA);
             } else {
                 const int cend = min(BN, a.Cout - n0);
+                float obj = -1.f, top = 0.f;
                 for (int c = 0; c < cend; c += 8) {
                     const uint4 q = *reinterpret_cast<const uint4 *>(row + c);
                     const int k = n0 + c;
-                    if (k + 8 <= a.hnc) store_scores8<false>(o + (size_t)(4 + k) * a.hA, (size_t)a.hA, q, 8);
-                    else store_scores8<true>(o + (size_t)(4 + k) * a.hA, (size_t)a.hA, q, a.hnc - k);
+                    const float2 s8 = k + 8 <= a.hnc ? store_scores8<false>(o + (size_t)(4 + k) * a.hA, (size_t)a.hA, q, 8)
+                                                     : store_scores8<true>(o + (size_t)(4 + k) * a.hA, (size_t)a.hA, q, a.hnc - k);
+                    if (k == 0) obj = s8.x;
+                    top = fmaxf(top, k == 0 ? s8.y : fmaxf(s8.x, s8.y));
+                }
+                if (a.hgate) {
+                    const int at = a.ha0 + i;
+                    uint32_t *w = a.hgate + (size_t)b * ((a.hA + 31) >> 5) + (at >> 5);
+                    if (obj >= a.hgate_thr) atomicOr(w, 1u << (at & 31));
+                    if (top >= a.hgate_thr) atomicOr(w + a.hgate_plane, 1u << (at & 31));
                 }
             }
         }
@@ -2573,7 +2560,8 @@
 
 static int conv1x1_head(rva_ctx *ctx, const void *in, int ldi, const void *weights, const float *bias, int batch, int H, int W,
                         int Cin, int Cout, int mode, void *out, float *boxes32, int nc, int anchors_total, int anchor_offset, float stride_px,
-                        int variant, rva_stream_t stream_, bool any_nc = false)
+                        int variant, rva_stream_t stream_, bool any_nc = false, uint32_t *gate = nullptr, float gate_thr = 0.f,
+                        int gate_plane = 0)
 {
     if (!ctx) return RVA_ERR_ARG;
     if (any_nc && (nc < 1 || nc > 1024 || anchor_offset < 0 || H <= 0 || W <= 0 || anchor_offset + H * W > anchors_total ||
@@ -2590,6 +2578,7 @@
     a.hout = (__half *)out; a.hmode = mode; a.hnc = nc; a.hA = anchors_total; a.ha0 = anchor_offset; a.hW = W; a.hHW = H * W;
     a.hstride = stride_px;
     a.hbox = boxes32;
+    if (mode == 2 && gate) { a.hgate = gate; a.hgate_thr = gate_thr; a.hgate_plane = gate_plane; }
     return launch_gather64_1x1<false, true>(ctx, "rva_conv1x1_head_f16", a, variant, (hipStream_t)stream_);
 }
 
@@ -2617,6 +2606,18 @@
     return conv1x1_head(ctx, in, ldi, weights, bias, batch, H, W, Cin, Cout, mode, out, boxes32, nc, anchors_total, anchor_offset, stride_px, variant,
                         stream_, true);
 }
+
+}
+
+int rva_conv1x1_head_gate_f16(rva_ctx *ctx, const void *in, int ldi, const void *weights, const float *bias, int batch, int H, int W,
+                              int Cin, int Cout, void *out, int nc, int anchors_total, int anchor_offset, float stride_px, int variant,
+                              uint32_t *gate, int gate_plane, float gate_thr, rva_stream_t stream_)
+{
+    return conv1x1_head(ctx, in, ldi, weights, bias, batch, H, W, Cin, Cout, 2, out, nullptr, nc, anchors_total, anchor_offset, stride_px, variant,
+                        stream_, true, gate, gate_thr, gate_plane);
+}
+
+extern "C" {
 
 int rva_conv1x1_head5_f16(rva_ctx *ctx, const void *in, int ldi, const void *weights, const float *bias, int batch, int H, int W,
                           int Cin, int nc, const float *anchors_px, void *out, float *boxes32, int anchors_total, int anchor_offset,
diff --git a/realtime_video_analytics_32streams_amd/csrc/rva_conv_dev.h b/realtime_video_analytics_32streams_amd/csrc/rva_conv_dev.h
--- a/realtime_video_analytics_32streams_amd/csrc/rva_conv_dev.h
+++ b/realtime_video_analytics_32streams_amd/csrc/rva_conv_dev.h
@@ -51,14 +51,59 @@
 template <int N> __device__ __forceinline__ void wait_vm() { asm volatile("s_waitcnt vmcnt(%0)" ::"n"(N) : "memory"); }
 
 template <bool GUARD>
-__device__ __forceinline__ void store_scores8(__half *o, size_t A, const uint4 q, int left)
+__device__ __forceinline__ float2 store_scores8(__half *o, size_t A, const uint4 q, int left)
 {
     const __half2 *hq = reinterpret_cast<const __half2 *>(&q);
+    float first = 0.f, top = 0.f;
 #pragma unroll
     for (int t = 0; t < 4; ++t) {
         const float2 f = __half22float2(hq[t]);
-        if (!GUARD || 2 * t < left) o[(size_t)(2 * t) * A] = __float2half_rn(__builtin_amdgcn_rcpf(1.0f + __expf(-f.x)));
-        if (!GUARD || 2 * t + 1 < left) o[(size_t)(2 * t + 1) * A] = __float2half_rn(__builtin_amdgcn_rcpf(1.0f + __expf(-f.y)));
+        if (!GUARD || 2 * t < left) {
+            const __half p = __float2half_rn(__builtin_amdgcn_rcpf(1.0f + __expf(-f.x)));
+            o[(size_t)(2 * t) * A] = p;
+            if (t == 0) first = __half2float(p);
+            else top = fmaxf(top, __half2float(p));
+        }
+        if (!GUARD || 2 * t + 1 < left) {
+            const __half p = __float2half_rn(__builtin_amdgcn_rcpf(1.0f + __expf(-f.y)));
+            o[(size_t)(2 * t + 1) * A] = p;
+            top = fmaxf(top, __half2float(p));
+        }
+    }
+    return make_float2(first, top);
+}
+
+__device__ __forceinline__ void head_box_decode(const __half *row, int i, int hW, float hstride, __half *o, float *o32, size_t A)
+{
+    float d[4];
+#pragma unroll
+    for (int sd = 0; sd < 4; ++sd) {
+        float v[16], mx = -1e30f;
+        const uint4 q0 = *reinterpret_cast<const uint4 *>(row + sd * 16), q1 = *reinterpret_cast<const uint4 *>(row + sd * 16 + 8);
+        const __half2 *h0 = reinterpret_cast<const __half2 *>(&q0), *h1 = reinterpret_cast<const __half2 *>(&q1);
+#pragma unroll
+        for (int t = 0; t < 4; ++t) {
+            float2 f = __half22float2(h0[t]); v[2 * t] = f.x; v[2 * t + 1] = f.y;
+            f = __half22float2(h1[t]); v[8 + 2 * t] = f.x; v[9 + 2 * t] = f.y;
+        }
+#pragma unroll
+        for (int t = 0; t < 16; ++t) mx = fmaxf(mx, v[t]);
+        float se = 0.f, sw = 0.f;
+#pragma unroll
+        for (int t = 0; t < 16; ++t) { const float e = __expf(v[t] - mx); se += e; sw += e * (float)t; }
+        d[sd] = sw / se;
+    }
+    const float ax = (float)(i % hW) + 0.5f, ay = (float)(i / hW) + 0.5f;
+    const float x1 = ax - d[0], y1 = ay - d[1], x2 = ax + d[2], y2 = ay + d[3];
+    o[0] = __float2half_rn((x1 + x2) * 0.5f * hstride);
+    o[A] = __float2half_rn((y1 + y2) * 0.5f * hstride);
+    o[2 * A] = __float2half_rn((x2 - x1) * hstride);
+    o[3 * A] = __float2half_rn((y2 - y1) * hstride);
+    if (o32) {
+        o32[0] = (x1 + x2) * 0.5f * hstride;
+        o32[A] = (y1 + y2) * 0.5f * hstride;
+        o32[2 * A] = (x2 - x1) * hstride;
+        o32[3 * A] = (y2 - y1) * hstride;
     }
 }
 
diff --git a/realtime_video_analytics_32streams_amd/csrc/rva_internal.h b/realtime_video_analytics_32streams_amd/csrc/rva_internal.h
--- a/realtime_video_analytics_32streams_amd/csrc/rva_internal.h
+++ b/realtime_video_analytics_32streams_amd/csrc/rva_internal.h
@@ -83,6 +83,18 @@
                             const void *residual, int ldr, int batch, int sel_batch, int H, int W, int Cin, int Cout, int ksize, int stride,
                             int act, int variant, int y0, int y1, rva_stream_t stream);
 
+int rva_conv1x1_head_gate_f16(rva_ctx *ctx, const void *in, int ldi, const void *weights, const float *bias, int batch, int H, int W,
+                              int Cin, int Cout, void *out, int nc, int anchors_total, int anchor_offset, float stride_px, int variant,
+                              uint32_t *gate, int gate_plane, float gate_thr, rva_stream_t stream);
+struct rva_box_tail_level {
+    const void *first; int ld;
+    int H, W, a0; float stride_px;
+    const void *w1; const float *b1;
+    const void *w2; const float *b2;
+};
+int rva_box_tail_f16(rva_ctx *ctx, const rva_box_tail_level *levels, const uint32_t *gate, int gate_plane, void *out, float *boxes32,
+                     int n, int nc, int anchors_total, rva_stream_t stream);
+
 void rva_jpeg_free(rva_ctx *ctx);
 
 
diff --git a/realtime_video_analytics_32streams_amd/csrc/rva_plan.hip b/realtime_video_analytics_32streams_amd/csrc/rva_plan.hip
--- a/realtime_video_analytics_32streams_amd/csrc/rva_plan.hip
+++ b/realtime_video_analytics_32streams_amd/csrc/rva_plan.hip
@@ -1,4 +1,5 @@
 #include <algorithm>
+#include <cmath>
 #include <cstring>
 #include <deque>
 #include <memory>
@@ -28,6 +29,7 @@
     int mode = 0, a0 = 0; float stride_px = 0.f;
     int c_real = 0;
     int Ho = 0, y0 = 0, y1 = 0;
+    bool gated = false;
     const void *hb[3] = {nullptr, nullptr, nullptr}, *hk[3] = {nullptr, nullptr, nullptr};
     int32_t hldb[3] = {0, 0, 0}, hldc[3] = {0, 0, 0}, hh[3] = {0, 0, 0}, hw[3] = {0, 0, 0}; float hs[3] = {0, 0, 0};
 };
@@ -54,6 +56,11 @@
     int rows_top = 0, rows_bottom = 0;
     bool windowed = false;
     int primed = 0;
+    bool tail_ok = false, gate_on = false;
+    float gate_thr = 0.f;
+    uint32_t *gate_map = nullptr;
+    int gate_words = 0;
+    rva_box_tail_level tail[3] = {};
 };
 
 namespace {
@@ -527,7 +534,17 @@
             const rva_conv_weights *sib[2] = {hd.box[l][0], cls[l][0]};
             if (!conv(sib, 2, feats[l], first, 3 + l, 1)) return false;
             if (!conv1(hd.box[l][1], first.sub(0, cb), b2, 3 + l, 1) || !head_last(hd, 3 + l, 1, hd.box[l][2], b2)) return false;
+            if (p->fused_head && cb == 64) {
+                Step &c1 = p->steps[p->steps.size() - 2], &h1 = p->steps.back();
+                c1.gated = h1.gated = true;
+                p->tail[l] = rva_box_tail_level{first.ptr(), first.ld, g.h[3 + l], g.w[3 + l], g.a0(3 + l), g.stride(3 + l), c1.w, c1.b, h1.w, h1.b};
+            }
             if (!conv1(cls[l][1], first.sub(cb, cc), k2, 3 + l, 1) || !head_last(hd, 3 + l, 2, cls[l][2], k2)) return false;
+        }
+        if (p->fused_head && cb == 64) {
+            p->gate_words = (p->A + 31) / 32;
+            p->gate_map = (uint32_t *)dev_alloc((size_t)2 * g.B * p->gate_words * sizeof(uint32_t), true);
+            p->tail_ok = p->gate_map != nullptr;
         }
         return head_close(hd);
     }
@@ -627,7 +644,11 @@
     case K_CONV: return rva_conv2d_nhwc_f16_sel(c, s.in, s.ldi, s.w, s.b, s.out, s.ldo, s.res, s.ldr, n, p->B, s.H, s.W, s.Cin, s.Cout, s.k, s.stride, s.act, variant,
                                                 0, -1, st);
     case K_UPCAT: return rva_conv1x1_upcat_f16(c, s.in, s.ldi, s.c_in, s.in2, s.ldi2, s.c_in2, s.w, s.b, s.out, s.ldo, n, s.H, s.W, s.Cout, s.act, variant, st);
-    case K_HEAD: return rva_conv1x1_head_nc_f16(c, s.in, s.ldi, s.w, s.b, n, s.H, s.W, s.Cin, s.Cout, s.mode, output, s.mode == 1 ? boxes : nullptr, p->nc,
+    case K_HEAD:
+        if (s.mode == 2 && p->gate_on)
+            return rva_conv1x1_head_gate_f16(c, s.in, s.ldi, s.w, s.b, n, s.H, s.W, s.Cin, s.Cout, output, p->nc, p->A, s.a0, s.stride_px, variant,
+                                             p->gate_map, p->B * p->gate_words, p->gate_thr, st);
+        return rva_conv1x1_head_nc_f16(c, s.in, s.ldi, s.w, s.b, n, s.H, s.W, s.Cin, s.Cout, s.mode, output, s.mode == 1 ? boxes : nullptr, p->nc,
                                                 p->A, s.a0, s.stride_px, variant, st);
     case K_PAIR32: return rva_c2f_pair32_f16(c, s.in, s.ldi, s.w, s.b, s.w2, s.b2, s.out, s.ldo, n, s.H, s.W, st);
     case K_STEM2: return rva_stem2_f16(c, input, s.w, s.b, s.w2, s.b2, s.out, s.ldo, n, s.H, s.W, st);
@@ -756,14 +777,32 @@
     return cs != hipStreamCaptureStatusNone;
 }
 
+int gate_clear(rva_yolov8_plan *p, int n, rva_stream_t stream)
+{
+    if (!p->gate_on) return RVA_OK;
+    (void)n;
+    RVA_HIP(p->ctx, hipMemsetAsync(p->gate_map, 0, (size_t)2 * p->B * p->gate_words * sizeof(uint32_t), (hipStream_t)stream));
+    return RVA_OK;
+}
+
+int gate_tail(rva_yolov8_plan *p, void *output, int n, rva_stream_t stream)
+{
+    if (!p->gate_on) return RVA_OK;
+    float *boxes = p->box32 ? (float *)((char *)output + p->box_off) : nullptr;
+    return rva_box_tail_f16(p->ctx, p->tail, p->gate_map, p->B * p->gate_words, output, boxes, n, p->nc, p->A, stream);
+}
+
 int run_steps(rva_yolov8_plan *p, const void *input, void *output, int n, int first, int last, rva_stream_t stream, bool win)
 {
+    if (first == 0 && first < last)
+        if (const int rc = gate_clear(p, n, stream); rc != RVA_OK) return rc;
     for (int i = first; i < last; ++i) {
         const Step &s = p->steps[i];
+        if (s.gated && p->gate_on) continue;
         const int rc = launch_step(p, s, s.variant, input, output, n, stream, win);
         if (rc != RVA_OK) return rc;
     }
-    return RVA_OK;
+    return first < last && last == (int)p->steps.size() ? gate_tail(p, output, n, stream) : RVA_OK;
 }
 
 int check_run(rva_yolov8_plan *p, const void *input, void *output, int n)
@@ -988,6 +1027,36 @@
     return RVA_OK;
 }
 
+int rva_box_gate_threshold_f16(double conf)
+{
+    if (!(conf >= 0x1p-24)) return 0;
+    if (conf >= 65504.0) return 0x7bff;
+    int e = 0;
+    (void)frexp(conf, &e);
+    e -= 1;
+    if (e < -14) return (int)floor(ldexp(conf, 24));
+    const int q = (int)floor(ldexp(conf, 10 - e));
+    return ((e + 15) << 10) | (q - 1024);
+}
+
+int rva_yolov8_plan_set_box_gate(rva_yolov8_plan *p, double conf)
+{
+    if (!p) return RVA_ERR_ARG;
+    const char *e = getenv("RVA_PLAN_NO_BOX_GATE");
+    if (e && e[0] == '1') return RVA_OK;
+    const bool on = p->tail_ok && conf > 0;
+    if (on != p->gate_on) p->primed = 0;
+    p->gate_on = on;
+    p->gate_thr = 0.f;
+    if (on) {
+        const int bits = rva_box_gate_threshold_f16(conf), ex = bits >> 10, m = bits & 1023;
+        p->gate_thr = ex ? ldexpf((float)(1024 + m), ex - 25) : ldexpf((float)m, -24);
+    }
+    return RVA_OK;
+}
+
+int rva_yolov8_plan_box_gate(const rva_yolov8_plan *p) { return p && p->gate_on ? 1 : 0; }
+
 int rva_yolov8_plan_step_rows(const rva_yolov8_plan *p, int step, int32_t *y0, int32_t *y1)
 {
     if (!p || step < 0 || step >= (int)p->steps.size()) return RVA_ERR_ARG;
@@ -1028,10 +1097,12 @@
     hipStream_t lanes[3] = {(hipStream_t)stream, (hipStream_t)side1, (hipStream_t)side2};
     bool started[3] = {true, false, false};
     const bool win = n <= p->primed;
+    if (const int rc = gate_clear(p, n, stream); rc != RVA_OK) return rc;
     for (int i = 0; i < (int)p->steps.size(); ++i) {
         for (int l = 1; l <= 2; ++l)
             if (p->fork_step[l] == i) RVA_HIP(p->ctx, hipEventRecord(p->fork_ev[l], lanes[0]));
         const Step &s = p->steps[i];
+        if (s.gated && p->gate_on) continue;
         if (s.lane && !started[s.lane]) {
             RVA_HIP(p->ctx, hipStreamWaitEvent(lanes[s.lane], p->fork_ev[s.lane], 0));
             started[s.lane] = true;
@@ -1044,6 +1115,7 @@
             RVA_HIP(p->ctx, hipEventRecord(p->join_ev[l], lanes[l]));
             RVA_HIP(p->ctx, hipStreamWaitEvent(lanes[0], p->join_ev[l], 0));
         }
+    if (const int rc = gate_tail(p, output, n, stream); rc != RVA_OK) return rc;
     note_complete_run(p, n, win, stream);
     return RVA_OK;
 }
diff --git a/realtime_video_analytics_32streams_amd/detector.py b/realtime_video_analytics_32streams_amd/detector.py
--- a/realtime_video_analytics_32streams_amd/detector.py
+++ b/realtime_video_analytics_32streams_amd/detector.py
@@ -110,6 +110,8 @@
                  seed: int = 0, device: Optional[int] = None):
         super().__init__(config)
         self._plans = {}
+        self._gate_told: dict = {}
+        self._gated = False
         self.ctx = ops.context(device)
         self.device = torch.device("cuda", self.ctx.device)
         if config.input_size:
@@ -218,9 +220,10 @@
 
     def invalidate_engine(self) -> None:
         self._plans.clear()
+        self._gate_told.clear()
         self._rows_told.clear()
 
-    def plan_for(self, tensor: torch.Tensor):
+    def plan_for(self, tensor: torch.Tensor, gate: Optional[bool] = None):
         batch = int(tensor.shape[0])
         shape = (self._images(batch), int(tensor.shape[2]), int(tensor.shape[3]))
         key = shape if self._slot == 0 else shape + (self._slot,)
@@ -234,11 +237,19 @@
             plan = self._plans[key] = plan_cls(self.net, shape[0], shape[1:], device=self.device, ctx=self.ctx,
                                                autotune=first is None, tune_overlap=getattr(self, "tune_overlap", 1),
                                                precision="fp32" if self.engine == "fused-f32" else "fp16", box_rows=self.box_rows,
-                                               static_rows=rows if self.engine == "fused" else None)
+                                               static_rows=rows if self.engine == "fused" else None,
+                                               box_gate=self._gate_conf(bool(gate)))
+            self._gate_told[key] = self._gate_conf(bool(gate))
             if first is not None:
                 plan.copy_tuning(first)
+        if gate is not None and self._gate_told.get(key) != self._gate_conf(gate):
+            plan.set_box_gate(self._gate_conf(gate))
+            self._gate_told[key] = self._gate_conf(gate)
         plan.n = batch
         return plan
+
+    def _gate_conf(self, gate: bool) -> float:
+        return float(self.config.confidence_threshold) if gate and self.engine == "fused" and self.arch == "yolov8" else 0.0
 
     def rows_pending(self, batch: int) -> bool:
         return not self._rows_told.get(self._buf_key(batch), True)
@@ -263,7 +274,7 @@
         if self.half:
             if tensor.dtype != torch.float16:
                 raise TypeError("half detector: the fused plan takes the fp16 tensor K1 writes")
-            plan = self.plan_for(tensor)
+            plan = self.plan_for(tensor, self._gated)
             if not torch.cuda.is_current_stream_capturing():
                 self._tell_rows(plan, tensor)
             plan(tensor.contiguous())
@@ -291,7 +302,11 @@
         return self._preprocess([p.frame for p in packets])
 
     def stage_net(self, pre):
-        return self._infer(pre[0])
+        self._gated = True
+        try:
+            return self._infer(pre[0])
+        finally:
+            self._gated = False
 
     def stage_post(self, raw, pre) -> ops.PostBuffers:
         return self._postprocess_device(raw, [pre[1]])
diff --git a/realtime_video_analytics_32streams_amd/engine.py b/realtime_video_analytics_32streams_amd/engine.py
--- a/realtime_video_analytics_32streams_amd/engine.py
+++ b/realtime_video_analytics_32streams_amd/engine.py
@@ -66,7 +66,7 @@
 
     def __init__(self, net: YoloV8, batch: int, hw: Tuple[int, int] = (640, 640), device: Optional[torch.device] = None,
                  ctx: Optional[N.Context] = None, autotune: bool = True, tune_overlap: int = 1, precision: str = "fp16",
-                 box_rows: str = "fp16", static_rows: Optional[Tuple[int, int]] = None):
+                 box_rows: str = "fp16", static_rows: Optional[Tuple[int, int]] = None, box_gate: Optional[float] = None):
         if precision not in ("fp16", "fp32"):
             raise ValueError(f"precision must be 'fp16' or 'fp32', not {precision!r}")
         if box_rows not in ("fp16", "fp32"):
@@ -109,6 +109,9 @@
         if static_rows is not None and tuple(static_rows) != (0, self.H) and os.environ.get("RVA_PLAN_NO_STATIC_ROWS") != "1":
             self.ctx.check(self.L.rva_yolov8_plan_set_static_rows(h, int(static_rows[0]), int(static_rows[1])), "rva_yolov8_plan_set_static_rows")
             self.static_rows = (int(static_rows[0]), int(static_rows[1]))
+        self.box_gate = 0.0
+        if box_gate:
+            self.set_box_gate(box_gate)
         info = [C.c_int32() for _ in range(5)]
         self.ctx.check(self.L.rva_yolov8_plan_info(h, *[C.byref(v) for v in info]), "rva_yolov8_plan_info")
         self.A, rows, self._n_steps, n_tun, self.quiet_step = (int(v.value) for v in info)
@@ -167,6 +170,10 @@
         self.static_rows = (int(top), int(bottom))
         self.rows_epoch += 1
         self._read_tunables()
+
+    def set_box_gate(self, conf: float) -> None:
+        self.ctx.check(self.L.rva_yolov8_plan_set_box_gate(self.handle, float(conf)), "rva_yolov8_plan_set_box_gate")
+        self.box_gate = float(conf) if int(self.L.rva_yolov8_plan_box_gate(self.handle)) else 0.0
 
     @property
     def primed_images(self) -> int:
```

After: 23780. About the same (-0.4%).
